# jpl-x/x_multi_agent

Measured on AMD Instinct MI355X. Metric: EKF updates/sec (window=30, 400 MSCKF feats), higher is better.
Workload: dtype f64; 1 GPU; BASELINE.json configs[3]: one agent per GPU, window N=30, K=400 MSCKF tracks (L=N), M=0 SLAM features, n=195; CI payload all-gather every 10 updates; n_poses_max=30, m_slam=0, agents=1, ci_every=10, payload_bytes=306072, ci_tracks_per_round=2, ci_rounds_rank0=0, ci_fused_rank0=0

## Files before the change

### include/xk.h

```cpp
#ifndef XK_H_
#define XK_H_

#ifdef __cplusplus
extern "C" {
#endif

typedef struct xk_handle xk_handle;

typedef enum {
  XK_OK = 0,
  XK_EINVAL = 1,
  XK_ESINGULAR = 2,
  XK_ENAN = 3,
  XK_EDEVICE = 4,
  XK_ENOMEM = 5,
  XK_ECAPACITY = 6
} xk_status;

#define XK_CORE 15


int xk_create(int device, int n_poses_max, int n_feat_max, int k_max, xk_handle **out);
int xk_destroy(xk_handle *h);
const char *xk_strerror(int status);
// ... 101 lines not shown
                       long tag);

int xk_pr_find_candidate(xk_pr *p, int uav_id, const unsigned char *query_vlad, double pr_score_thr, int *index,
                         double *score, long *tag);

int xk_pr_keyframe(xk_pr *p, int index, const double **d_payload, const double **d_tracks, int *n_desc, long *tag,
                   unsigned char *desc_out);

int xk_pr_copy_keyframe(xk_pr *p, int index, double *d_payload_dst, double *d_tracks_dst);

int xk_pr_knn_match(xk_pr *p, const unsigned char *query, int nq, const unsigned char *train, int nt, int *idx, int *dist);

int xk_pr_essential_ransac(xk_pr *p, const float *cur_xy, const float *rec_xy, int n, double fx, double fy, double cx,
                           double cy, double threshold_px, int n_hyp, unsigned long seed, unsigned char *mask,
                           double *E , int *n_inliers);

int xk_pr_essential_hypotheses(xk_pr *p, int first, int count, int *n_cand, double *E ,
                               int *inliers );

typedef struct xk_trk xk_trk;

int xk_trk_create(xk_handle *h, int max_matches, double fx, double fy, double cx, double cy, double s, xk_trk **out);
void xk_trk_destroy(xk_trk *t);

int xk_trk_undistort(xk_trk *t, const double *dist_xy, int n, double *xy);

int xk_trk_fundamental_ransac(xk_trk *t, const float *prev_xy, const float *cur_xy, int n, double threshold_px, int n_hyp,
                              unsigned long seed, unsigned char *mask, double *F ,
                              int *n_inliers);

int xk_trk_fundamental_hypotheses(xk_trk *t, int first, int count, int *n_cand, double *F ,
                                  int *inliers );

int xk_trk_filter_matches(xk_trk *t, const double *prev_dist_xy, const double *cur_dist_xy, int n, double threshold_px,
                          int n_hyp, unsigned long seed, unsigned char *mask, int *keep_idx, double *prev_xy, double *cur_xy,
                          int *n_inliers);


int xk_trk_klt_setup(xk_trk *t, int width, int height, int win_w, int win_h, int max_level, int max_iter, double eps,
                     double min_eig_thr);
int xk_trk_klt_levels(xk_trk *t);

int xk_trk_push_image(xk_trk *t, const unsigned char *img, int stride);

int xk_trk_track(xk_trk *t, const float *prev_xy, int n, double *cur_xy, unsigned char *status, double *min_eig, int *keep_idx,
                 double *kept_prev_xy, double *kept_cur_xy, int *n_kept);

int xk_trk_klt_level(xk_trk *t, int which, int level, unsigned char *img, short *dIx, short *dIy, int *w, int *h);

int xk_build_compress_async(xk_handle *h, double sigma_img);

int xk_build_compress_update_async(xk_handle *h, double sigma_img);

int xk_build_compress_update_pass_async(xk_handle *h, double sigma_img, const double *corr_total, int cov_update);
int xk_fetch_flags(xk_handle *h, int *inlier_msckf, double *gamma_msckf, int *inlier_slam, double *gamma_slam);


int xk_stage_range(xk_handle *h, double range, double img_x_n, double img_y_n, const int facet[3], double sigma_range);
int xk_stage_sun_angle(xk_handle *h, const double q_xyzw[4], double x_angle_deg, double y_angle_deg, const double *calib);
int xk_fetch_aux_flags(xk_handle *h, int *range_inlier, double *range_gamma);
int xk_aux_rows(xk_handle *h, double *H, int ldh, double *res, double *r_diag, int *rows);

int xk_apply_ci_resident(xk_handle *h, const double *ci_P, int ldc, int n, const double *H, int ldh, int m,
                         const double *res, const double *S, int lds, double *correction);

int xk_snapshot_P(xk_handle *h, int restore);


#define XK_NSTAGE 6
typedef struct {
  float total_ms;
  float stage_ms[XK_NSTAGE];
  int stage_launches[XK_NSTAGE];
  char stage_name[XK_NSTAGE][32];
  int n, c1, k_tracks, rows_stacked, n_leaf, n_levels;
} xk_timing;

int xk_bench_staged(xk_handle *h, double sigma_img, int warmup, int steps, xk_timing *out);

int xk_run_steps(xk_handle *h, double sigma_img, int steps);

int xk_caqr_status(const xk_handle *h, int *schedule, int *armed, int *giveups, int *last_reason);

int xk_set_option(xk_handle *h, const char *name, int value);

#ifdef __cplusplus
}
#endif
#endif
```

### x_multi_agent_amd/csrc/xk_api.hip

```cpp
#include "../../include/xk.h"
#ifdef XK_LAB
#include "../../include/xk_lab.h"
#endif

#include <hip/hip_runtime.h>

#include <algorithm>
#include <cmath>
#include <cstdio>
#include <cstdlib>
#include <cstring>
#include <functional>
#include <vector>

#include "xk_chi2_table.h"
#include "xk_feature.hip.h"
#include "xk_slaminit.hip.h"
#include "xk_linalg.hip.h"
#include "xk_caqr_pipe.hip.h"
#include "xk_ci.hip.h"
#include "xk_ciw.hip.h"
#include "xk_ciw_round.hip.h"
#include "xk_aux.hip.h"

// ... 54 lines not shown
  h->CM = round_up(h->n + 1 + 3, 16);
  h->LDA = h->CM + round_up(h->n + 1, 16);
  HIPCHK(h, hipSetDevice(device));
  HIPCHK(h, hipStreamCreateWithFlags(&h->stream, hipStreamNonBlocking));
  HIPCHK(h, hipStreamCreateWithFlags(&h->copy_stream, hipStreamNonBlocking));
  HIPCHK(h, hipEventCreateWithFlags(&h->ev_flags, hipEventDisableTiming));
  HIPCHK(h, hipEventCreateWithFlags(&h->ev_flags_done, hipEventDisableTiming));
  for (auto &e : h->ev) HIPCHK(h, hipEventCreate(&e));
  const size_t nn = (size_t)h->n * h->n;
  h->obs_cap = (size_t)k_max * n_poses_max;
  HIPCHK(h, dalloc(&h->d_q, 7 * (size_t)n_poses_max));
  HIPCHK(h, hipMalloc((void **)&h->d_done_cnt, sizeof(unsigned)));
  HIPCHK(h, hipMemset(h->d_done_cnt, 0, sizeof(unsigned)));
  h->h_win = (double *)calloc(7 * (size_t)n_poses_max, sizeof(double));
  if (!h->h_win) return fail(h, XK_EDEVICE, "host allocation");
  h->d_p = h->d_q + 4 * (size_t)n_poses_max;
  HIPCHK(h, dalloc(&h->d_obs, 2 * h->obs_cap + ((size_t)k_max + 2) / 2 + 1));
  h->d_trk_off = (int *)(h->d_obs + 2 * h->obs_cap);
  HIPCHK(h, dalloc(&h->d_feat, 3 * (size_t)n_feat_max));
  HIPCHK(h, dalloc(&h->d_zlast, 2 * (size_t)n_feat_max));
  HIPCHK(h, dalloc(&h->d_anchor, (size_t)n_feat_max));
  HIPCHK(h, dalloc(&h->d_tsz, (size_t)n_feat_max));
  HIPCHK(h, dalloc(&h->d_P, nn));
  HIPCHK(h, dalloc(&h->d_Pout, nn));
  HIPCHK(h, dalloc(&h->d_fq, (size_t)450));
  HIPCHK(h, dalloc(&h->d_chi95, (size_t)XK_CHI2_LEN));
  HIPCHK(h, dalloc(&h->d_chi90, (size_t)XK_CHI2_LEN));
  HIPCHK(h, hipMemcpy(h->d_chi95, XK_CHI2_095, sizeof(double) * XK_CHI2_LEN, hipMemcpyHostToDevice));
  HIPCHK(h, hipMemcpy(h->d_chi90, XK_CHI2_090, sizeof(double) * XK_CHI2_LEN, hipMemcpyHostToDevice));
  HIPCHK(h, dalloc(&h->d_A, ((size_t)h->ntiles_max * h->DB + 256) * h->C1P));
  HIPCHK(h, hipMemset(h->d_A + (size_t)h->ntiles_max * h->DB * h->C1P, 0, sizeof(double) * 256 * h->C1P));
  h->hc_stride = xk_hc_stride(h->DB, h->C1P);
  h->opt_hlite = env_int("XK_HLITE", 1);
  h->rows_compact = false;
  HIPCHK(h, dalloc(&h->d_Hc, (size_t)std::max(k_max, 1) * h->hc_stride));
  HIPCHK(h, dalloc(&h->d_tile_rows, (size_t)h->ntiles_max));
  for (auto &pp : h->d_panel) HIPCHK(h, dalloc(&pp, (size_t)(h->ntiles_max + 10) * 256));
  HIPCHK(h, dalloc(&h->d_inl, (size_t)k_max));
  HIPCHK(h, dalloc(&h->d_inl_s, (size_t)n_feat_max));
  HIPCHK(h, dalloc(&h->d_gn, (size_t)k_max));
  HIPCHK(h, dalloc(&h->d_gam, (size_t)k_max));
  HIPCHK(h, dalloc(&h->d_gam_s, (size_t)n_feat_max));
  HIPCHK(h, dalloc(&h->d_gpf, 3 * (size_t)k_max));
  HIPCHK(h, dalloc(&h->d_R, (size_t)h->C1P * h->C1P));
  HIPCHK(h, hipMemset(h->d_R, 0, sizeof(double) * (size_t)h->C1P * h->C1P));
  HIPCHK(h, dalloc(&h->d_R2, (size_t)(h->C1P + 32) * h->C1P));
  HIPCHK(h, hipMemset(h->d_R2, 0, sizeof(double) * (size_t)(h->C1P + 32) * h->C1P));
  {
    hipDeviceProp_t prop;
    HIPCHK(h, hipGetDeviceProperties(&prop, device));
    h->n_cu = prop.multiProcessorCount;
    h->persist_ok = h->DB == 64 && h->C1 <= XkPipeWide::COLS && h->n_cu == 256;
    if (h->persist_ok) {
      int nb1 = 0;
      const void *kfn = h->C1 <= XkPipeNarrow::COLS ? (const void *)xk_caqr_pipe<XkPipeNarrow> : (const void *)xk_caqr_pipe<XkPipeWide>;
      if (hipOccupancyMaxActiveBlocksPerMultiprocessor(&nb1, kfn, XK_PIPE_THREADS, 0) != hipSuccess) nb1 = 0;
      h->persist_ok = nb1 >= 1;
      if (h->persist_ok && h->C1 <= XkPipeNarrow::COLS) {
        int nb2 = 0;
        if (hipOccupancyMaxActiveBlocksPerMultiprocessor(&nb2, (const void *)xk_caqr_pipe<XkPipeNarrow2>, XK_PIPE_THREADS, 0) != hipSuccess) nb2 = 0;
        if (nb2 < 1) h->opt_split = -1;
      }
      (void)hipGetLastError();
    }
    h->fast_capable = h->persist_ok;
    h->tail_capable = h->DB == 128 && h->n_cu == 256 && h->C1 > 32;
    if (h->tail_capable) {
      int nbt = 0, nbt4 = 0;
      if (hipOccupancyMaxActiveBlocksPerMultiprocessor(&nbt, (const void *)xk_caqr_pipe<XkPipeTail>, XK_PIPE_THREADS, 0) != hipSuccess) nbt = 0;
      if (hipOccupancyMaxActiveBlocksPerMultiprocessor(&nbt4, (const void *)xk_caqr_pipe<XkPipeTail4>, XK_PIPE_THREADS, 0) != hipSuccess) nbt4 = 0;
      h->tail_capable = nbt >= 1 && nbt4 >= 1;
      (void)hipGetLastError();
    }
    h->tail_ok = h->tail_capable;
    h->opt_tail = env_int("XK_CAQR_TAIL", 1);
    h->opt_slam_split = env_int("XK_SLAM_SPLIT", 1);
    h->opt_pipe_min_rows = env_int("XK_PIPE_MIN_ROWS", 1);
    h->rearm_after = env_int("XK_CAQR_REARM", 64);
    h->opt_resident = env_int("XK_CAQR_RESIDENT", 1);
    h->opt_poison = env_int("XK_CAQR_RESIDENT_POISON", 0);
    h->opt_test_stall = env_int("XK_CAQR_TEST_STALL", 0);
    h->opt_tall26 = env_int("XK_CAQR_TALL26", 1);
    h->opt_kalman = env_int("XK_PIPE_KALMAN", 1);
    if (h->opt_split >= 0) h->opt_split = env_int("XK_PIPE_SPLIT", 1);
    if (!h->fast_capable && h->DB == 64 && h->C1 <= XkPipeWide::COLS) {
      snprintf(h->err, sizeof(h->err), "single-launch CAQR unavailable on device %d: %s; the multi-launch schedule serves every update",
               device, h->n_cu != 256 ? "the process does not see 256 compute units (partition mode or CU mask)"
                                      : "a 768-thread workgroup of the kernel does not fit a compute unit");
      static const int quiet = env_int("XK_QUIET", 0);
      if (!quiet) fprintf(stderr, "xk: %s (n_cu = %d)\n", h->err, h->n_cu);
    }
    if (h->persist_ok || h->tail_capable) {
      const size_t np = h->persist_ok ? (size_t)(h->C1 + 15) / 16 : (size_t)XkPipeTail4::COLS / 16, strips = np * XK_PIPE_RLS;
      h->xslab_doubles = strips * 16 * h->C1P * 2 + strips * 256;
      HIPCHK(h, dalloc(&h->d_x1, 2 * h->xslab_doubles));
      HIPCHK(h, hipMemsetD32Async((hipDeviceptr_t)h->d_x1, (int)(XK_NOTYET_BITS & 0xffffffffu), 2 * 2 * h->xslab_doubles, h->stream));
      HIPCHK(h, dalloc(&h->d_rs, (size_t)8 * XK_PIPE_NT_MAX * 16 * h->C1P));
      HIPCHK(h, dalloc(&h->d_rpb, (size_t)8 * XK_PIPE_NT_MAX * 256));
      HIPCHK(h, dalloc(&h->d_xsync, (size_t)2 * XP_WORDS * 16));
      HIPCHK(h, hipMemset(h->d_xsync, 0, sizeof(unsigned) * 2 * XP_WORDS * 16));
      h->xsync_phase = 0;
#ifdef XK_LAB
      HIPCHK(h, dalloc(&h->d_pdbg, (size_t)XK_PDBG_WORDS));
      HIPCHK(h, hipMemset(h->d_pdbg, 0, sizeof(long long) * XK_PDBG_WORDS));
#endif
    }
  }
  HIPCHK(h, dalloc(&h->d_Maug, (size_t)h->CM * h->LDA));
  HIPCHK(h, dalloc(&h->d_X, (size_t)h->CM * h->LDA));
  HIPCHK(h, dalloc(&h->d_corr, (size_t)h->n + 4));
  HIPCHK(h, dalloc(&h->d_ct, (size_t)h->n));
  HIPCHK(h, dalloc(&h->d_tmpH, (size_t)h->CM * h->n));
  HIPCHK(h, dalloc(&h->d_tmpS, (size_t)h->CM * h->CM));
  HIPCHK(h, dalloc(&h->d_tmpP, nn));
  HIPCHK(h, dalloc(&h->d_rdiag, (size_t)h->CM));
  HIPCHK(h, dalloc(&h->d_tmpz, (size_t)h->CM));
  HIPCHK(h, dalloc(&h->d_aux, 3 * ((size_t)h->n + 1) + 8));
  HIPCHK(h, dalloc(&h->d_Taug, (size_t)h->CM * ((size_t)h->n + 2)));
  HIPCHK(h, hipHostMalloc((void **)&h->h_out, sizeof(double) * ((size_t)h->n + 4), hipHostMallocDefault));
  memset(h->h_out, 0, sizeof(double) * ((size_t)h->n + 4));
  h->d_status = (int *)(h->h_out + h->n);
  HIPCHK(h, dalloc(&h->d_payload, (size_t)xk_payload_doubles(n_poses_max, n_feat_max)));
  HIPCHK(h, dalloc(&h->d_ci, (size_t)4 * nn + 64 * (size_t)h->n + 1024));
  HIPCHK(h, dalloc(&h->d_ciw, (size_t)XK_CIW_WS));
  h->h_pin_doubles = nn + 8 * (size_t)h->n + 4 * (size_t)k_max + 4 * (size_t)n_feat_max + 1024;
  HIPCHK(h, hipHostMalloc((void **)&h->h_pin, sizeof(double) * h->h_pin_doubles));
  h->csr_cap = 24 * (size_t)h->n + 3 * (size_t)n_feat_max * h->n;
  {
    const size_t m = (size_t)std::max(n_feat_max, 1);
    HIPCHK(h, dalloc(&h->d_trk2_off, m + 1));
    HIPCHK(h, dalloc(&h->d_inl2, m));
    HIPCHK(h, dalloc(&h->d_gn2, m));
    HIPCHK(h, dalloc(&h->d_obs2, 2 * m * n_poses_max));
    HIPCHK(h, dalloc(&h->d_gpf2, 3 * m));
    HIPCHK(h, dalloc(&h->d_W2, m * h->DB * h->na));
    HIPCHK(h, dalloc(&h->d_gam2, m));
    HIPCHK(h, dalloc(&h->d_H1, 3 * m * h->n));
    HIPCHK(h, dalloc(&h->d_H2, 9 * m));
    HIPCHK(h, dalloc(&h->d_r1, 3 * m));
    HIPCHK(h, dalloc(&h->d_feat2, 3 * m));
    h->h_trk2_off = (int *)calloc(m + 1, sizeof(int));
    if (!h->h_trk2_off) return fail(h, XK_ENOMEM, "host track offsets");
  }
  HIPCHK(h, dalloc(&h->d_csr_v, h->csr_cap + XK_CORE * XK_CORE + 9 * (size_t)n_feat_max * n_feat_max + 7 * (size_t)n_poses_max + ((size_t)h->n + 2 + h->csr_cap) / 2 + 1));
  h->d_csr_i = nullptr;
  h->h_trk_off = (int *)calloc((size_t)k_max + 1, sizeof(int));
  if (!h->h_trk_off) return fail(h, XK_ENOMEM, "host track offsets");
  HIPCHK(h, hipHostMalloc((void **)&h->h_pin_i, sizeof(int) * ((size_t)k_max + n_feat_max + 512)));
  h->stage_bytes = std::max({sizeof(double) * 2 * h->obs_cap + sizeof(int) * ((size_t)k_max + 1), sizeof(double) * 7 * (size_t)n_poses_max,
                             (sizeof(int) + sizeof(double)) * h->csr_cap + sizeof(int) * ((size_t)h->n + 1) + sizeof(double) * (XK_CORE * XK_CORE + 9 * (size_t)n_feat_max * n_feat_max + 7 * (size_t)n_poses_max),
                             sizeof(double) * 8 * (size_t)std::max(n_feat_max, 1)}) + 256;
  for (auto &sp : h->h_stage) HIPCHK(h, hipHostMalloc((void **)&sp, h->stage_bytes));

  HIPCHK(h, hipHostMalloc((void **)&h->h_flag_i, sizeof(int) * ((size_t)k_max + n_feat_max + 8)));
  HIPCHK(h, hipHostMalloc((void **)&h->h_flag_d, sizeof(double) * ((size_t)k_max + n_feat_max + 8)));
  memset(h->d_status, 0, sizeof(int) * 4);
  HIPCHK(h, hipMemset(h->d_tile_rows, 0, sizeof(int) * (size_t)h->ntiles_max));
  h->sigma_img = 0.0;
  *out = h;
  return XK_OK;
}

extern "C" int xk_destroy(xk_handle *h) {
  if (!h) return XK_OK;
  hipSetDevice(h->device);
  hipStreamSynchronize(h->stream);
// ... 1942 lines not shown
    hipError_t e = hipStreamEndCapture(h->stream, &g);
    if (rc != XK_OK) return rc;
    if (e != hipSuccess) return fail(h, XK_EDEVICE, "graph capture", e);
    HIPCHK(h, hipGraphInstantiate(&ge, g, nullptr, nullptr, 0));
    for (int it = 0; it < steps; ++it) HIPCHK(h, hipGraphLaunch(ge, h->stream));
    rc = read_status(h);
    hipGraphExecDestroy(ge);
    hipGraphDestroy(g);
    return rc;
  }
#endif
  for (int attempt = 0; attempt < 2; ++attempt) {
    for (int it = 0; it < steps; ++it) {
      int rc = launch_build(h, sigma_img, attempt > 0 || it > 0);
      if (rc != XK_OK) return rc;
      UpdateSpec u = compressed_spec(h, nullptr, 1);
      rc = launch_compress(h, nullptr, &u);
      if (rc != XK_OK) return rc;
      if (!h->last.fused) rc = launch_update(h, u);
      if (rc != XK_OK) return rc;
    }
    const int rc = read_status(h, attempt == 0);
    if (rc != XK_RETRY_CLASSIC) return rc;
  }
  return XK_EDEVICE;
}

#ifdef XK_LAB
__global__ __launch_bounds__(256) void xk_probe_mfma(double *out, int iters) {
  xk_d4 a0 = {0, 0, 0, 0}, a1 = a0, a2 = a0, a3 = a0;
  const double x = 1.0 + threadIdx.x * 1e-9, y = 1.0 - threadIdx.x * 1e-9;
  for (int i = 0; i < iters; ++i) {
    a0 = __builtin_amdgcn_mfma_f64_16x16x4f64(x, y, a0, 0, 0, 0);
    a1 = __builtin_amdgcn_mfma_f64_16x16x4f64(y, x, a1, 0, 0, 0);
    a2 = __builtin_amdgcn_mfma_f64_16x16x4f64(x, x, a2, 0, 0, 0);
    a3 = __builtin_amdgcn_mfma_f64_16x16x4f64(y, y, a3, 0, 0, 0);
  }
  out[(size_t)blockIdx.x * blockDim.x + threadIdx.x] = a0[0] + a1[1] + a2[2] + a3[3];
}
__global__ __launch_bounds__(256) void xk_probe_fma(double *out, int iters) {
  double a[8];
  const double x = 1.0 + threadIdx.x * 1e-9, y = 1e-9 * threadIdx.x;
#pragma unroll
  for (int k = 0; k < 8; ++k) a[k] = k;
  for (int i = 0; i < iters; ++i) {
#pragma unroll
    for (int k = 0; k < 8; ++k) a[k] = fma(a[k], x, y);
  }
  double s = 0;
#pragma unroll
  for (int k = 0; k < 8; ++k) s += a[k];
  out[(size_t)blockIdx.x * blockDim.x + threadIdx.x] = s;
}

extern "C" int xk_probe_fp64_peak(xk_handle *h, int use_mfma, double *tflops) {
  if (!h || !tflops) return XK_EINVAL;
  HIPCHK(h, hipSetDevice(h->device));
  const int blocks = 256 * 8, iters = 20000;
  double *buf = nullptr;
  HIPCHK(h, hipMalloc((void **)&buf, sizeof(double) * blocks * 256));
  for (int rep = 0; rep < 2; ++rep) {
    HIPCHK(h, hipEventRecord(h->ev[8], h->stream));
    if (use_mfma) hipLaunchKernelGGL(xk_probe_mfma, dim3(blocks), dim3(256), 0, h->stream, buf, iters);
    else hipLaunchKernelGGL(xk_probe_fma, dim3(blocks), dim3(256), 0, h->stream, buf, iters);
    HIPCHK(h, hipEventRecord(h->ev[9], h->stream));
    HIPCHK(h, hipStreamSynchronize(h->stream));
  }
  float ms = 0;
  hipEventElapsedTime(&ms, h->ev[8], h->ev[9]);
  hipFree(buf);
  const double waves = (double)blocks * 4;
  const double flops = use_mfma ? waves * iters * 4.0 * (2.0 * 16 * 16 * 4) : waves * 64.0 * iters * 8.0 * 2.0;
  *tflops = flops / (ms * 1e-3) / 1e12;
  return XK_OK;
}
#endif

extern "C" int xk_set_option(xk_handle *h, const char *name, int value) {
  if (!h || !name) return XK_EINVAL;
  if (!strcmp(name, "caqr_resident")) h->opt_resident = value;
  else if (!strcmp(name, "caqr_rearm")) h->rearm_after = value;
  else if (!strcmp(name, "caqr_tail")) h->opt_tail = value;
  else if (!strcmp(name, "slam_split")) h->opt_slam_split = value;
  else if (!strcmp(name, "ci_weight_search")) {
    if (value != 0 && value != 1) return fail(h, XK_EINVAL, "xk_set_option: ci_weight_search is 0 or 1");
    h->opt_ci_search = value;
  }
#ifdef XK_LAB
  else if (!strcmp(name, "caqr_poison")) h->opt_poison = value;
  else if (!strcmp(name, "caqr_test_stall")) h->opt_test_stall = value;
  else if (!strcmp(name, "caqr_tall26")) h->opt_tall26 = value;
  else if (!strcmp(name, "pipe_kalman")) h->opt_kalman = value;
  else if (!strcmp(name, "pipe_split")) { if (h->opt_split >= 0) h->opt_split = value; }
  else if (!strcmp(name, "caqr_hlite")) h->opt_hlite = value;
#endif
  else return fail(h, XK_EINVAL, "xk_set_option: unknown option");
  return XK_OK;
}

extern "C" int xk_caqr_status(const xk_handle *h, int *schedule, int *armed, int *giveups, int *last_reason) {
  if (!h) return XK_EINVAL;
  if (schedule) *schedule = outcome_status(h->last);
  if (armed) *armed = (h->persist_ok || h->tail_ok) ? 1 : 0;
  if (giveups) *giveups = h->fast_giveups;
  if (last_reason) *last_reason = h->fast_reason;
  return XK_OK;
}

#ifdef XK_LAB
extern "C" int xk_is_lab(void) { return 1; }
extern "C" int xk_debug_persist_stamps(xk_handle *h, long long *out, int n_out) {
  if (!h || !out || !h->d_pdbg) return XK_EINVAL;
  HIPCHK(h, hipSetDevice(h->device));
  HIPCHK(h, hipStreamSynchronize(h->stream));
  HIPCHK(h, hipMemcpy(out, h->d_pdbg, sizeof(long long) * (size_t)std::min(n_out, XK_PDBG_WORDS), hipMemcpyDeviceToHost));
  return XK_OK;
}
extern "C" int xk_debug_feature_points(xk_handle *h, double *gpf, int *gn_iters, int K) {
  if (!h || !gpf || !gn_iters || K < 0 || K != h->K) return XK_EINVAL;
  HIPCHK(h, hipSetDevice(h->device));
  HIPCHK(h, hipStreamSynchronize(h->stream));
  if (K == 0) return XK_OK;
  HIPCHK(h, hipMemcpy(gpf, h->d_gpf, sizeof(double) * 3 * (size_t)K, hipMemcpyDeviceToHost));
  HIPCHK(h, hipMemcpy(gn_iters, h->d_gn, sizeof(int) * (size_t)K, hipMemcpyDeviceToHost));
  return XK_OK;
}
#endif

#if defined(XK_FEAT_PROBE) && defined(XK_LAB)
extern "C" int xk_debug_feature_phases(xk_handle *h, double sigma_img, long long *out, int n_out) {
  const size_t bytes = sizeof(long long) * (size_t)(12 * h->K);
  hipMalloc((void **)&h->feat_dbg, bytes);
  hipMemset(h->feat_dbg, 0, bytes);
  int rc = launch_build(h, sigma_img);
  hipStreamSynchronize(h->stream);
  hipMemcpy(out, h->feat_dbg, std::min(bytes, sizeof(long long) * (size_t)n_out), hipMemcpyDeviceToHost);
  hipFree(h->feat_dbg);
  h->feat_dbg = nullptr;
  return rc;
}
#endif

#include "xk_place.hip.h"
#include "xk_essential.hip.h"

#define XK_PR_MAX_KEYFRAMES 15

struct xk_pr {
  xk_handle *h;
  int k, L, n_nodes, kmax, W, n_words, clusters, VW, max_desc;
  long pay_n, trk_n;
  unsigned int *d_node_desc;
  int *d_children, *d_word_of_node, *d_node_of_word;
  unsigned int *d_vlad;
  unsigned int *d_kfdesc;
  double *d_payload;
  double *d_tracks;
  int n_desc[XK_PR_MAX_KEYFRAMES];
  long tag[XK_PR_MAX_KEYFRAMES];
  std::vector<int> *uav_ids[XK_PR_MAX_KEYFRAMES];
  int order[XK_PR_MAX_KEYFRAMES], live;
  unsigned int *d_q, *d_t, *d_qvlad;
  int *d_ham, *d_knn;
  int *h_int;
  unsigned int *h_words;
  size_t h_words_cap;
  double *d_ess;
  unsigned char *h_ess;
  int ess_n_hyp;
};

#define XK_ESS_OFF_SUM ((size_t)XK_ESS_MAX_HYP * XK_ESS_MAXC * 9)
#define XK_ESS_OFF_E (XK_ESS_OFF_SUM + (size_t)XK_ESS_MAX_HYP * XK_ESS_MAXC)
#define XK_ESS_OFF_KEY (XK_ESS_OFF_E + 9)
#define XK_ESS_DOUBLES (XK_ESS_OFF_KEY + 1)
#define XK_ESS_INTS ((size_t)XK_ESS_MAX_HYP * (XK_ESS_MAXC + 2) + 2)

extern "C" void xk_pr_destroy(xk_pr *p) {
  if (!p) return;
  hipFree(p->d_node_desc); hipFree(p->d_children); hipFree(p->d_word_of_node); hipFree(p->d_node_of_word);
  hipFree(p->d_vlad); hipFree(p->d_kfdesc); hipFree(p->d_payload); hipFree(p->d_tracks);
  hipFree(p->d_q); hipFree(p->d_t); hipFree(p->d_qvlad); hipFree(p->d_ham); hipFree(p->d_knn);
  if (p->h_int) hipHostFree(p->h_int);
  if (p->h_words) hipHostFree(p->h_words);
  hipFree(p->d_ess);
  if (p->h_ess) hipHostFree(p->h_ess);
  for (auto &u : p->uav_ids) delete u;
  free(p);
}

// ... 675 lines not shown
```

### x_multi_agent_amd/csrc/xk_caqr_pipe.hip.h

```cpp
#pragma once
#include <hip/hip_runtime.h>

#include <type_traits>

#include "xk_linalg.hip.h"
#include "xk_xcd_sync.hip.h"

#define XK_PIPE_THREADS 768
#ifndef XK_PIPE_NPH
#define XK_PIPE_NPH 4
#endif
template <int LPC_, int RPL_, int NT_, int NM_, int NCL_, int NCM_ = 1, int RPLS_ = RPL_, int RPLT_ = RPLS_, int NG_ = 1, int NPH_ = XK_PIPE_NPH>
struct XkPipeGeom {
  static constexpr int LPC = LPC_, RPL = RPL_, NT = NT_, NM = NM_, NCL = NCL_, NCM = NCM_, NG = NG_;
  static constexpr int NPH = NPH_;
  static_assert(NPH_ == 1 || NPH_ == 2 || NPH_ == 4, "XP_TQ_CNT / XP_X1_CNT hold four phases");
  static constexpr int NTG = (NT_ + NG_ - 1) / NG_, NMG = NM_ / NG_;
  static_assert(NM_ % NG_ == 0 && NG_ >= 1 && NG_ <= 2, "first-level groups share the first-level workgroups evenly");
  static constexpr int RPLS = RPLS_, RPLT = RPLT_;
  static_assert(RPLS_ % 4 == 0 && RPLS_ >= 16 && RPLS_ <= RPL_ && RPLT_ % 4 == 0 && RPLT_ >= 16 && RPLT_ <= RPLS_, "the lighter tile steps");
  static constexpr int RM = (NTG + 2) & ~1;
  static constexpr int RL = 8 * NG_;
  static constexpr int COLS = XK_PIPE_THREADS / LPC_;
  static constexpr int ROWS = 8 * NT_ * LPC_ * RPL_;
// ... 15 lines not shown
#ifndef XK_PIPE_TAIL
#define XK_PIPE_TAIL 8, 44, 23, 8, 1, 1, 44, 44, 1, 4
#endif
using XkPipeTail = XkPipeGeom<XK_PIPE_TAIL>;
#ifndef XK_PIPE_TAIL4
#define XK_PIPE_TAIL4 4, 44, 23, 8, 1, 1, 44, 44, 1, 4
#endif
using XkPipeTail4 = XkPipeGeom<XK_PIPE_TAIL4>;
#define XK_PIPE_RLS 16
#define XK_PIPE_NT_MAX 23
#define XK_PIPE_ROWS_MAX 24320
#define XK_PIPE_SLOTS_MAX 1536
#ifndef XK_PIPE_PB
#define XK_PIPE_PB 0, 4, 8, 12, 16
#endif
#ifndef XK_PIPE_PB2
#define XK_PIPE_PB2 0, 8, 16
#endif
template <int NPH>
__host__ __device__ constexpr int xk_pbn(int q) {
  if (NPH == 4) {
    constexpr int t[] = {XK_PIPE_PB};
    return q <= 0 ? 0 : (q >= 4 ? 16 : t[q]);
  }
  if (NPH == 2) {
    constexpr int t[] = {XK_PIPE_PB2};
    return q <= 0 ? 0 : (q >= 2 ? 16 : t[q]);
  }
  return q * (16 / NPH);
}
#ifndef XK_PIPE_ARRD
#define XK_PIPE_ARRD 1
#endif
#ifndef XK_PIPE_PF
#define XK_PIPE_PF 0
#endif
#ifndef XK_PIPE_LOCALLD
#define XK_PIPE_LOCALLD 0
#endif
#if XK_PIPE_LOCALLD
#define XK_LD_LOC(p) xk_ld_grp(p)
#ifdef XK_PIPE_NOINV
#define XK_INV_LOC()
#else
#define XK_INV_LOC() xk_inv_l1()
#endif
#else
#define XK_LD_LOC(p) xk_ld_sc1(p)
#define XK_INV_LOC()
#endif
#ifndef XK_PIPE_TRI
#define XK_PIPE_TRI 0
#endif
#ifndef XK_PIPE_NLW
#define XK_PIPE_NLW 7
#endif
#ifndef XK_PIPE_CHUNK
#define XK_PIPE_CHUNK 0
#endif

enum {
  XP_CENSUS = 0,
  XP_ABORT = 9,
  XP_TQ_CNT = 16,
  XP_MB_CNT = 48,
  XP_X1_CNT = 64,
  XP_P_CNT = 64 + 4 * XK_CAQR_MAXP,
  XP_R_CNT = 64 + 5 * XK_CAQR_MAXP,
  XP_WORDS = 64 + 6 * XK_CAQR_MAXP
};

struct XkCaqrPipeArgs {
  const double *A;
  const double *Hc;
  int hs, nhc;
  const int *tile_rows;
  int nslots;
  int slot_rows;
  int lead_stride;
  int res_col;
  int nextra;
  long extra_row0;
  int C1P, C1;
  double *Rout;
  double *S;
  double *PB;
  double *X1, *X1P;
  double *X2;
  double *Xnext;
  long xnext_doubles;
  unsigned *sync, *sync_next;
  int *status;
  long long *dbg;
  int test_stall;
  int acc_tag;
  int kal, kn;
  const double *Pin;
  double *Pout;
  double sigma2;
  double *corr;
  const double *ct;
  unsigned long long *done_flag;
  unsigned long long done_seq;
};
typedef const XkCaqrPipeArgs __attribute__((address_space(4))) *XkPipeArgsPtr;
__device__ __forceinline__ XkCaqrPipeArgs xk_pipe_args(XkPipeArgsPtr ap) {
  XkCaqrPipeArgs a;
  __builtin_memcpy(&a, (const void *)ap, sizeof(a));
  return a;
}

__device__ __forceinline__ void xk_pipe_arrive(unsigned *cnt) {
  (void)__hip_atomic_fetch_add(cnt, 1u, XK_ARRIVE_ORDER, __HIP_MEMORY_SCOPE_AGENT);
}
__device__ __forceinline__ int xk_launder(int v) {
  asm volatile("" : "+v"(v));
  return v;
}
__device__ __forceinline__ size_t xk_blk(int c, int r) { return (size_t)(c >> 2) * 64 + (size_t)r * 4 + (size_t)(c & 3); }
__device__ __forceinline__ int xk_pipe_srccol(const XkCaqrPipeArgs &a, int c) { return (a.res_col > 0 && c == a.C1 - 1) ? a.res_col : c; }
__device__ __forceinline__ void xk_pipe_lastcut(int trail, int NCL, int &ncl, int &lchalf, int &lsplit) {
  ncl = (NCL > 1 && trail > 32 * XK_PIPE_NLW) ? NCL : 1;
  lchalf = max(4, 4 * ((trail + 4 * XK_PIPE_NLW * ncl - 1) / (4 * XK_PIPE_NLW * ncl)));
  lsplit = max(1, (trail + lchalf - 1) / lchalf);
}
__device__ __forceinline__ bool xk_pipe_wait(unsigned *word, unsigned target, unsigned *ab, unsigned reason, unsigned *s_ok) {
  if (threadIdx.x == 0) *s_ok = xk_spin_ge(word, target, ab, reason) ? 1u : 0u;
  __syncthreads();
  const bool ok = *s_ok != 0u;
  XK_ACQUIRE_FENCE();
  __syncthreads();
  return ok;
}

__device__ __forceinline__ int xk_pipe_wait_phases(unsigned *cnt0, int stride, int q, int nph, unsigned target, unsigned *ab, unsigned reason,
                                                   unsigned *s_ok) {
  if (threadIdx.x == 0) {
    unsigned av = 0;
    if (xk_spin_ge(cnt0 + (size_t)q * stride, target, ab, reason)) {
      av = (unsigned)q + 1u;
      while ((int)av < nph && __hip_atomic_load(cnt0 + (size_t)av * stride, XK_RLX_AGENT) >= target) ++av;
    }
    *s_ok = av;
  }
  __syncthreads();
  const int av = (int)*s_ok;
  XK_ACQUIRE_FENCE();
  __syncthreads();
  return av;
}

template <int KK, int LPC, int RPL>
__device__ __forceinline__ void xk_pipe_tapply(double (&b)[RPL], int rel, bool live, int part, const double *ubuf, const double *sc) {
  if constexpr (XK_PIPE_CHUNK || RPL > 32) {
    constexpr int RPLP = RPL + 2, H = RPL / 4;
    constexpr int pb = KK & 1;
    const xk_d2 *useg = reinterpret_cast<const xk_d2 *>(ubuf + (pb * LPC + part) * RPLP);
    const double mtt = sc[pb * 4];
    if (rel > KK && live && mtt != 0.0) {
      double d0 = 0.0, d1 = 0.0, d2 = 0.0, d3 = 0.0;
      {
        xk_d2 u[H];
#pragma unroll
        for (int r = 0; r < H; ++r) u[r] = useg[r];
#pragma unroll
        for (int r = 0; r < H; ++r) {
          if (r & 1) { d2 = fma(u[r][0], b[2 * r], d2); d3 = fma(u[r][1], b[2 * r + 1], d3); }
          else { d0 = fma(u[r][0], b[2 * r], d0); d1 = fma(u[r][1], b[2 * r + 1], d1); }
        }
      }
      xk_d2 v[H];
#pragma unroll
      for (int r = 0; r < H; ++r) v[r] = useg[H + r];
#pragma unroll
      for (int r = 0; r < H; ++r) {
        if ((H + r) & 1) { d2 = fma(v[r][0], b[2 * (H + r)], d2); d3 = fma(v[r][1], b[2 * (H + r) + 1], d3); }
        else { d0 = fma(v[r][0], b[2 * (H + r)], d0); d1 = fma(v[r][1], b[2 * (H + r) + 1], d1); }
      }
      const double w = mtt * xk_group_sum<LPC>((d0 + d1) + (d2 + d3));
#pragma unroll
      for (int r = 0; r < H; ++r) {
        b[2 * (H + r)] = fma(w, v[r][0], b[2 * (H + r)]);
        b[2 * (H + r) + 1] = fma(w, v[r][1], b[2 * (H + r) + 1]);
      }
      const xk_d2 *useg2 = useg + xk_launder(0);
#pragma unroll
      for (int r = 0; r < H; ++r) {
        const xk_d2 u = useg2[r];
        b[2 * r] = fma(w, u[0], b[2 * r]);
        b[2 * r + 1] = fma(w, u[1], b[2 * r + 1]);
      }
    }
  } else {
// ... 144 lines not shown
struct XkNoStepHook { __device__ __forceinline__ void operator()(int) const {} };
template <int LPC, int K, int K1, int KH, int RPL, typename Hook, typename Every>
__device__ __forceinline__ void xk_pipe_range_it(double (&b)[RPL], double (*b2)[RPL], int rel, bool live, bool live2, int part, int nsteps,
                                                 double *ubuf, double *sc, bool hook_on, Hook hook, Every every) {
  if constexpr (K < K1) {
    if (K < nsteps) {
      xk_pipe_apply2<LPC, K - 1, RPL>(b, b2, rel, live, live2, part, ubuf, sc);
      xk_pipe_form<LPC, K, RPL>(b, rel, part, ubuf, sc);
      if (K == KH && hook_on) asm volatile("s_waitcnt vmcnt(0)" ::: "memory");
      __syncthreads();
      if (K == KH && hook_on && threadIdx.x == 0) hook();
      every(K);
    } else if (K == nsteps) {
      xk_pipe_apply2<LPC, K - 1, RPL>(b, b2, rel, live, live2, part, ubuf, sc);
    }
    xk_pipe_range_it<LPC, K + 1, K1, KH, RPL>(b, b2, rel, live, live2, part, nsteps, ubuf, sc, hook_on, hook, every);
  }
}
template <int LPC, int K0, int K1, int KH, int RPL, typename Hook, typename Every>
__device__ __forceinline__ void xk_pipe_range(double (&b)[RPL], double (*b2)[RPL], int rel, bool live, bool live2, int part, int nsteps,
                                              double *ubuf, double *sc, bool hook_on, Hook hook, Every every) {
  if (K0 < nsteps) xk_pipe_form<LPC, K0, RPL>(b, rel, part, ubuf, sc);
  if (KH == K0 && hook_on) asm volatile("s_waitcnt vmcnt(0)" ::: "memory");
  __syncthreads();
  if (KH == K0 && hook_on && threadIdx.x == 0) hook();
  every(K0);
  xk_pipe_range_it<LPC, K0 + 1, K1, KH, RPL>(b, b2, rel, live, live2, part, nsteps, ubuf, sc, hook_on, hook, every);
  if (nsteps >= K1) xk_pipe_apply2<LPC, K1 - 1, RPL>(b, b2, rel, live, live2, part, ubuf, sc);
}
template <int LPC, int K0, int K1, int KH, int RPL, typename Hook>
__device__ __forceinline__ void xk_pipe_range(double (&b)[RPL], double (*b2)[RPL], int rel, bool live, bool live2, int part, int nsteps,
                                              double *ubuf, double *sc, bool hook_on, Hook hook) {
  xk_pipe_range<LPC, K0, K1, KH, RPL>(b, b2, rel, live, live2, part, nsteps, ubuf, sc, hook_on, hook, XkNoStepHook());
}

template <class G>
__device__ __forceinline__ int xk_pipe_rowplan(const XkCaqrPipeArgs &a, int j, int *pre, int *myrows, int *rows_accepted) {
  constexpr int NTP = 8 * G::NT, CAP = G::LPC * G::RPL;
  const int tid = threadIdx.x, lane = tid & 63, wave = tid >> 6;
  __shared__ int wsum[XK_PIPE_THREADS / 64];
  int carry = 0;
  for (int base = 0; base < a.nslots; base += XK_PIPE_THREADS) {
    const int t = base + tid;
    int v = t < a.nslots ? a.tile_rows[t] : 0;
    if (a.lead_stride > 0 && t < a.nslots && t % a.lead_stride == 0) v = max(v, 32);
#pragma unroll
    for (int o = 1; o < 64; o <<= 1) {
      const int u = __shfl_up(v, o, 64);
      if (lane >= o) v += u;
    }
    if (lane == 63) wsum[wave] = v;
    __syncthreads();
    int off = carry;
    for (int w = 0; w < wave; ++w) off += wsum[w];
    if (t < a.nslots) pre[t + 1] = v + off;
    int tot = 0;
    for (int w = 0; w < XK_PIPE_THREADS / 64; ++w) tot += wsum[w];
    carry += tot;
    __syncthreads();
  }
  if (tid == 0) pre[0] = 0;
  const int Rs = carry, R = Rs + a.nextra, TR = (R + NTP - 1) / NTP;
  *rows_accepted = R;
  __syncthreads();
  if (TR > CAP) return 0;
  if (tid < CAP) {
    const int g = j * TR + tid;
    int phys = -1;
    if (tid < TR && g >= Rs && g < R) phys = (int)a.extra_row0 + (g - Rs);
    else if (tid < TR && g < Rs) {
      int lo = 0, hi = a.nslots;
      while (hi - lo > 1) {
        const int mid = (lo + hi) >> 1;
        if (pre[mid] <= g) lo = mid; else hi = mid;
      }
      phys = lo * a.slot_rows + (g - pre[lo]);
    }
    myrows[tid] = phys;
  }
  __syncthreads();
  return max(TR, 1);
}

template <class G, int RPL>
__device__ __noinline__ bool xk_pipe_tile(XkPipeArgsPtr ap, int xcc, int slot, long long t_entry, double *ubuf, double *sc, unsigned *s_ok,
                                          const int *myrows, double *hbuf, int hcap_doubles, int nvalid) {
  constexpr int NT = G::NT, LPC = G::LPC, NPH = G::NPH, GS = 16 / NPH, ARRD = XK_PIPE_ARRD;
  static_assert(ARRD < xk_pbn<NPH>(1) && ARRD < 16 - xk_pbn<NPH>(NPH - 1), "a phase is counted in before the next one is published");
  const XkCaqrPipeArgs a = xk_pipe_args(ap);
  unsigned *sync = a.sync, *ab = sync + XP_ABORT * 16;
  const int tid = threadIdx.x;
  const int j = xcc * NT + slot;
  const int cabs = tid / LPC, part_ = tid % LPC;
  const bool mine = cabs < a.C1;
  const int npanels = (a.C1 + 15) / 16;
  const bool stamp = a.dbg && xcc == 0 && slot == 1 && tid == 0;
  double b[RPL];
  if (a.nhc > 0) {
    constexpr int BR = 8, CG = XK_PIPE_THREADS / LPC;
    const int hs = a.hs, C1P = a.C1P, ccl = min(cabs, C1P - 1);
    double *Tb = hbuf, *recs = hbuf + LPC * BR * C1P;
    const int hcap = (hcap_doubles - LPC * BR * C1P) / hs;
#pragma unroll
    for (int r = 0; r < RPL; ++r) b[r] = 0.0;
    if (stamp) a.dbg[1544] = wall_clock64();
    const int s_lo = myrows[0] >> 6, s_hi = nvalid > 0 ? myrows[nvalid - 1] >> 6 : -1;
    const int fp = __builtin_amdgcn_readfirstlane(tid / CG), fc = tid % CG;
    if (stamp) a.dbg[1545] = wall_clock64();
    for (int lo = max(s_lo, 0); lo <= s_hi && lo < a.nhc; lo += hcap) {
      const int hi = min(min(lo + hcap, s_hi + 1), a.nhc);
      {
        const xk_d2 *src = reinterpret_cast<const xk_d2 *>(a.Hc + (size_t)lo * hs);
        xk_d2 *dst = reinterpret_cast<xk_d2 *>(recs);
        const int tot = (hi - lo) * (hs / 2);
        for (int base = 0; base < tot; base += 6 * XK_PIPE_THREADS) {
          xk_d2 t[6];
#pragma unroll
          for (int i = 0; i < 6; ++i) t[i] = src[min(base + i * XK_PIPE_THREADS + tid, tot - 1)];
#pragma unroll
          for (int i = 0; i < 6; ++i) {
            const int e = base + i * XK_PIPE_THREADS + tid;
            if (e < tot) dst[e] = t[i];
          }
        }
      }
      __syncthreads();
      if (stamp) a.dbg[1546] = wall_clock64();
      int kcur = -1, r0 = -2;
      double nw0 = 0.0, nw1 = 0.0, nw2 = 0.0, wres = 0.0, x0 = 0.0, x1 = 0.0;
      const bool whole = lo <= s_lo && s_hi < hi;
#pragma unroll
      for (int rb = 0; rb < (RPL + BR - 1) / BR; ++rb) {
        if (fc < C1P) {
#pragma unroll
          for (int j = 0; j < BR; ++j) {
            if (rb * BR + j < RPL) {
              const int ph = __builtin_amdgcn_readfirstlane(myrows[fp * RPL + rb * BR + j]), sl = ph >> 6;
              if (ph >= 0 && sl >= lo && sl < hi) {
                const double *rec = recs + (sl - lo) * hs;
                if (sl != kcur) {
                  const xk_d2 *wc = reinterpret_cast<const xk_d2 *>(rec + XK_HC_VR + XK_HC_WC * xk_pipe_srccol(a, fc));
                  const xk_d2 q0 = wc[0], q1 = wc[1], q2 = wc[2];
                  nw0 = -q0[0]; nw1 = -q0[1]; nw2 = -q1[0]; x0 = q1[1]; x1 = q2[0]; r0 = (int)q2[1];
                  wres = (r0 == -1) ? 1.0 : 0.0;
                  kcur = sl;
                }
                const int rr = (ph & 63) + 3, dd = rr - r0;
                const xk_d2 va = reinterpret_cast<const xk_d2 *>(rec + 4 * rr)[0], vb = reinterpret_cast<const xk_d2 *>(rec + 4 * rr)[1];
                const double add = (dd == 0) ? x0 : ((dd == 1) ? x1 : 0.0);
                Tb[(fp * BR + j) * C1P + fc] = fma(wres, vb[1], fma(nw2, vb[0], fma(nw1, va[1], nw0 * va[0]))) + add;
              }
            }
          }
        }
        __syncthreads();
        if (whole) {
#pragma unroll
          for (int j = 0; j < BR; ++j) {
            if (rb * BR + j < RPL) {
              const double v = Tb[(part_ * BR + j) * C1P + ccl];
              b[rb * BR + j] = (mine && part_ * RPL + rb * BR + j < nvalid) ? v : 0.0;
            }
          }
        } else {
#pragma unroll
          for (int j = 0; j < BR; ++j) {
            if (rb * BR + j < RPL) {
              const int ph = myrows[part_ * RPL + rb * BR + j], sl = ph >> 6;
              const double v = Tb[(part_ * BR + j) * C1P + ccl];
              if (ph >= 0 && sl >= lo && sl < hi) b[rb * BR + j] = mine ? v : 0.0;
            }
          }
        }
        __syncthreads();
        if (stamp) a.dbg[1547 + rb] = wall_clock64();
      }
    }
    if (s_hi >= a.nhc) {
      const double *Ac = a.A + xk_pipe_srccol(a, ccl);
#pragma unroll
      for (int h0 = 0; h0 < RPL; h0 += 16) {
        double x[16];
#pragma unroll
        for (int r = 0; r < 16; ++r) {
          if (h0 + r < RPL) x[r] = Ac[(size_t)max(myrows[part_ * RPL + h0 + r], 0) * C1P];
        }
#pragma unroll
        for (int r = 0; r < 16; ++r) {
          if (h0 + r < RPL) {
            const int ph = myrows[part_ * RPL + h0 + r];
            if (mine && ph >= 0 && (ph >> 6) >= a.nhc) b[h0 + r] = x[r];
          }
        }
      }
    }
  } else
  {
    int pr[RPL];
#pragma unroll
    for (int r = 0; r < RPL; ++r) pr[r] = myrows[part_ * RPL + r];
    const double *Ac = a.A + xk_pipe_srccol(a, min(cabs, a.C1P - 1));
#pragma unroll
    for (int h0 = 0; h0 < RPL; h0 += 16) {
      double x[16];
#pragma unroll
      for (int r = 0; r < 16; ++r) {
        if (h0 + r < RPL) x[r] = Ac[(size_t)max(pr[h0 + r], 0) * a.C1P];
      }
#pragma unroll
      for (int r = 0; r < 16; ++r) {
        if (h0 + r < RPL) b[h0 + r] = (mine && pr[h0 + r] >= 0) ? x[r] : 0.0;
      }
    }
  }
  double *myS = a.S + (size_t)j * 16 * a.C1P;
  double *myPB = a.PB + (size_t)j * 256;
  if (stamp) { a.dbg[1536] = t_entry; a.dbg[1537] = wall_clock64(); }
  for (int k = 0; k < npanels; ++k) {
    const int c0 = 16 * k;
    const int part = xk_launder(part_);
    const int rel = xk_launder(cabs) - c0;
    const int nsteps = (a.C1 - c0 < 16) ? a.C1 - c0 : 16;
    const bool full = nsteps == 16;
    const int wrel = (tid >> 6) * (64 / LPC) - c0;
    const bool hot = wrel <= 0 && wrel > -(64 / LPC);
    const bool pub = mine && part == 0 && rel >= 0;
    const unsigned epoch = (unsigned)(k + 1);
    if (stamp) { a.dbg[16 * k + 0] = wall_clock64(); a.dbg[16 * k + 8] = clock64(); }
    if (a.dbg && slot == 0 && tid == 0) a.dbg[12288 + xcc * 32 + k] = wall_clock64();
    if (a.dbg && tid == 0 && k < 2) a.dbg[40960 + 256 * k + j] = wall_clock64();
    if (a.dbg && tid == 0 && k == 0) a.dbg[40960 + 512 + j] = t_entry;
    if (hot) __builtin_amdgcn_s_setprio(3);
    auto phase = [&](auto qc) {
      constexpr int q = decltype(qc)::value;
      auto hook = [&]() { xk_pipe_arrive(sync + (XP_TQ_CNT + (q - 1) * 8 + xcc) * 16); if (a.dbg && k == 0 && q == 1) a.dbg[47104 + j] = wall_clock64(); };
      xk_pipe_range<LPC, xk_pbn<NPH>(q), xk_pbn<NPH>(q + 1), (q > 0 ? xk_pbn<NPH>(q) + ARRD : -1), RPL>(b, nullptr, rel, mine, false, part, nsteps, ubuf, sc, full, hook);
      if (pub) {
        if (rel < 16) {
          double *pb = xk_opaque(myPB + xk_blk(rel, 0));
#pragma unroll
          for (int r = xk_pbn<NPH>(q); r < xk_pbn<NPH>(q + 1); ++r) pb[r * 4] = (r > rel) ? 0.0 : b[r];
        } else {
          double *ps = xk_opaque(myS + xk_blk(cabs, 0));
#pragma unroll
          for (int r = xk_pbn<NPH>(q); r < xk_pbn<NPH>(q + 1); ++r) ps[r * 4] = b[r];
        }
      }
      if (stamp && q < 4) a.dbg[16 * k + 1 + q] = wall_clock64();
    };
    phase(std::integral_constant<int, 0>{});
    if constexpr (NPH >= 2) phase(std::integral_constant<int, 1>{});
    if constexpr (NPH >= 4) { phase(std::integral_constant<int, 2>{}); phase(std::integral_constant<int, 3>{}); }
    if constexpr (NPH >= 8) {
      phase(std::integral_constant<int, 4>{}); phase(std::integral_constant<int, 5>{});
      phase(std::integral_constant<int, 6>{}); phase(std::integral_constant<int, 7>{});
    }
    if (hot) __builtin_amdgcn_s_setprio(0);
    if (stamp) { a.dbg[16 * k + 9] = clock64(); a.dbg[16 * k + 10] = wall_clock64(); }
    asm volatile("s_waitcnt vmcnt(0)" ::: "memory");
    __syncthreads();
    if (tid == 0) {
      for (int q = full ? NPH - 1 : 0; q < NPH; ++q)
        xk_pipe_arrive(sync + (XP_TQ_CNT + q * 8 + xcc) * 16);
    }
    if (stamp) a.dbg[16 * k + 5] = wall_clock64();
    if (k + 1 == npanels) break;
    if (!xk_pipe_wait(sync + (XP_MB_CNT + xcc) * 16, (unsigned)G::NM * epoch, ab, 2u, s_ok)) return false;
    if (stamp) a.dbg[16 * k + 6] = wall_clock64();
    XK_INV_LOC();
    if (mine && rel >= 16 && part == 0) {
      const double *ps = xk_opaque(myS + xk_blk(cabs, 0));
#pragma unroll
      for (int r = 0; r < 16; ++r) b[r] = XK_LD_LOC(ps + r * 4);
    }
    if (stamp) {
      double sink = 0;
      for (int r = 0; r < 16; ++r) sink += b[r];
      asm volatile("" ::"v"(sink));
      a.dbg[16 * k + 7] = wall_clock64();
    }
  }
  if (stamp) a.dbg[1538] = wall_clock64();
  return true;
}

__device__ __forceinline__ void xk_lds_dma16(const double *src, unsigned lds_byte) {
  asm volatile("s_mov_b32 m0, %1\n\tglobal_load_lds_dwordx4 %0, off sc1" ::"v"(src), "s"(lds_byte) : "memory", "m0");
}

template <class G>
__device__ __noinline__ bool xk_pipe_first(XkPipeArgsPtr ap, int xcc, int item, double *ubuf, double *sc, unsigned *s_ok, double *pfbuf) {
  constexpr int NT = G::NT, NM = G::NMG, RM = G::RM, NP = 16, NPH = G::NPH, GS = 16 / NPH, NCL = G::NCL, NCM = G::NCM;
  constexpr int NG = G::NG, NTG = G::NTG;
  const XkCaqrPipeArgs a = xk_pipe_args(ap);
  unsigned *sync = a.sync, *ab = sync + XP_ABORT * 16;
  const int tid = threadIdx.x;
  const int cidx_ = tid / NP, part_ = tid & (NP - 1);
  const bool panel = cidx_ < 16;
  const int npanels = (a.C1 + 15) / 16;
  const int grp = NG > 1 ? item / NM : 0;
  item -= grp * NM;
  const int nts = NG > 1 ? min(NTG, NT - grp * NTG) : NT;
  const int base = xcc * NT + grp * NTG;
  const bool has_pending = !(xcc == 0 && grp == 0);
  const size_t SS = (size_t)16 * a.C1P;
  const bool stamp = a.dbg && xcc == 0 && item == 0 && tid == 0;
  for (int k = 0; k < npanels; ++k) {
    const int c0 = 16 * k, trail = max(0, a.C1 - c0 - 16);
    const int cidx = xk_launder(cidx_), part = xk_launder(part_);
    const int mh = min(32, 4 * ((trail + 4 * NM * NCM - 1) / (4 * NM * NCM))), mch = mh * NCM;
    const bool active = item == 0 || item * mch < trail;
    const int col = panel ? c0 + cidx : c0 + 16 + item * mch + (cidx - 16);
    const int col2 = col + mh;
    const bool mine = active && col < a.C1 && (panel || cidx - 16 < mh);
    const bool mine2 = NCM > 1 && active && !panel && cidx - 16 < mh && col2 < a.C1;
    const int nsteps = (a.C1 - c0 < 16) ? a.C1 - c0 : 16;
    const bool full = nsteps == 16;
    const unsigned epoch = (unsigned)(k + 1);
    const size_t slab = (size_t)k * XK_PIPE_RLS + xcc * NG + grp;
    double b[RM], b2[NCM > 1 ? RM : 2];
    b[0] = 0.0;
    b2[0] = 0.0;
    int ncl_prev, lchalf_prev, lsplit_prev;
    xk_pipe_lastcut(a.C1 - c0, NCL, ncl_prev, lchalf_prev, lsplit_prev);
    lsplit_prev = min(XK_PIPE_NLW, lsplit_prev);
    const size_t pslab = (size_t)(k - 1) * XK_PIPE_RLS + xcc * NG + grp;
    if (k >= 1 && has_pending) {
#if XK_DATA_POLL
      double pb1[1] = {0.0}, pb2[1] = {0.0};
      if (!xk_poll_slots<1>(pb1, a.X2 + pslab * SS + xk_blk(min(col, a.C1P - 1), part), 0, mine, ab, 4u)) *s_ok = 0u;
      if constexpr (NCM > 1) {
        if (!xk_poll_slots<1>(pb2, a.X2 + pslab * SS + xk_blk(min(col2, a.C1P - 1), part), 0, mine2, ab, 4u)) *s_ok = 0u;
      }
      __syncthreads();
      if (*s_ok == 0u) return false;
      if (mine) b[0] = pb1[0];
      if constexpr (NCM > 1) b2[0] = mine2 ? pb2[0] : 0.0;
      if (a.dbg && tid == 0) a.dbg[4096 + ((xcc * NG + grp) * NM + item) * 32 + k] = wall_clock64();
#else
      if (!xk_pipe_wait(sync + (XP_P_CNT + k - 1) * 16, (unsigned)lsplit_prev, ab, 4u, s_ok)) return false;
      if (mine) b[0] = xk_ld_sc1(a.X2 + pslab * SS + xk_blk(col, part));
#endif
    }
#pragma unroll
    for (int s = 1; s < RM; ++s) b[s] = 0.0;
    if constexpr (NCM > 1) {
#pragma unroll
      for (int s = 1; s < RM; ++s) b2[s] = 0.0;
#if !XK_DATA_POLL
      if (k >= 1 && has_pending && mine2) b2[0] = xk_ld_sc1(a.X2 + pslab * SS + xk_blk(col2, part));
#endif
    }
    double *g02 = a.S + (size_t)base * SS + xk_blk(min(col2, a.C1P - 1), part);
    double *x12 = a.X1 + slab * SS + xk_blk(min(col2, a.C1P - 1), part);
    const size_t lane_off = panel ? xk_blk(cidx, part) : xk_blk(col, part);
    const size_t strip_step = panel ? 256 : SS;
    double *g0 = (panel ? a.PB + (size_t)base * 256 : a.S + (size_t)base * SS) + lane_off;
    double *x1 = panel ? a.X1P + slab * 256 + xk_blk(cidx, part) : a.X1 + slab * SS + xk_blk(col, part);
    const bool x1_mine = mine && (!panel || item == 0);
    bool ok = true;
    int loaded = 0;
    constexpr bool PF = XK_PIPE_PF && NG == 1 && NCM == 1 && NPH == 4 && NT <= 24 && xk_pbn<NPH>(1) == 4 && xk_pbn<NPH>(2) == 8 && xk_pbn<NPH>(3) == 12;
    const int ln = tid & 63, cid4 = cidx & ~3;
    const int wcol = panel ? c0 + cid4 : c0 + 16 + item * mch + (cid4 - 16);
    const bool wv_ok = active && (panel || cid4 - 16 < mh) && wcol < a.C1;
    double *pfw = pfbuf + (size_t)(tid >> 6) * (24 * 16);
    const unsigned pfw_lds = (unsigned)__builtin_amdgcn_readfirstlane((int)(unsigned)(size_t)pfw);
    const double *pfsrc = (panel ? a.PB + (size_t)base * 256 + xk_blk(cid4, 0) : a.S + (size_t)base * SS + xk_blk(wcol, 0)) +
                          (size_t)(ln >> 3) * strip_step + (ln & 7) * 2;
    auto phase = [&](auto qc) {
      constexpr int q = decltype(qc)::value;
      if (!ok) return;
#ifdef XK_PIPE_PROBE_M1PACE
      if (q > 0 && loaded > q) {
        if (xk_pipe_wait_phases(sync + (XP_TQ_CNT + xcc) * 16, 8 * 16, q, NPH, (unsigned)NT * epoch, ab, 6u, s_ok) == 0) { ok = false; return; }
      }
#endif
      if (loaded <= q) {
#ifdef XK_PIPE_PROBE_M1ALL
        int av = xk_pipe_wait_phases(sync + (XP_TQ_CNT + xcc) * 16, 8 * 16, q, NPH, (unsigned)NT * epoch, ab, 6u, s_ok);
        if (av != 0) av = NPH;
#else
        const int av = xk_pipe_wait_phases(sync + (XP_TQ_CNT + xcc) * 16, 8 * 16, q, NPH, (unsigned)NT * epoch, ab, 6u, s_ok);
#endif
        if (av == 0) { ok = false; return; }
        if (stamp && q < 4) a.dbg[512 + 16 * k + 2 * q] = wall_clock64();
        if (a.dbg && tid == 0 && k == 0 && q == 0) a.dbg[46080 + (xcc * NG + grp) * NM + item] = wall_clock64();
        XK_INV_LOC();
        if constexpr (PF) {
          for (int p = loaded; p < av; ++p) {
            if (wv_ok) {
              const double *src = pfsrc + (size_t)p * 16;
#pragma unroll
              for (int j = 0; j < 3; ++j)
                if (8 * j + (ln >> 3) < NT) xk_lds_dma16(src + (size_t)(8 * j) * strip_step, pfw_lds + (unsigned)j * 1024u);
              asm volatile("s_waitcnt vmcnt(0)" ::: "memory");
              if (mine && part >= p * GS && part < (p + 1) * GS) {
                typedef const __attribute__((address_space(3))) double xk_lds_cd;
                xk_lds_cd *pl = (xk_lds_cd *)(pfw + (part - p * GS) * 4 + (cidx & 3));
#pragma unroll
                for (int s = 1; s <= NT; ++s) b[s] = pl[(s - 1) * 16];
              }
              if (p + 1 < av) asm volatile("s_waitcnt lgkmcnt(0)" ::: "memory");
            }
          }
        } else {
          if (active && mine && part >= xk_pbn<NPH>(loaded) && part < xk_pbn<NPH>(av)) {
            double *g = xk_opaque(g0);
#pragma unroll
            for (int s = 1; s <= NTG; ++s)
              if (NG == 1 || s <= nts) b[s] = XK_LD_LOC(g + (size_t)(s - 1) * strip_step);
          }
        }
        if constexpr (NCM > 1) {
          if (mine2 && part >= xk_pbn<NPH>(loaded) && part < xk_pbn<NPH>(av)) {
            double *g = xk_opaque(g02);
#pragma unroll
            for (int s = 1; s <= NTG; ++s)
              if (NG == 1 || s <= nts) b2[s] = xk_ld_sc1(g + (size_t)(s - 1) * SS);
          }
        }
        loaded = av;
#ifdef XK_PIPE_M1PROBE
        asm volatile("s_waitcnt vmcnt(0)" ::: "memory");
        if (stamp && q < 4) a.dbg[512 + 16 * k + 10 + q] = wall_clock64();
#endif
      }
      if (!active) return;
      if (panel) __builtin_amdgcn_s_setprio(3);
      auto hook = [&]() { xk_pipe_arrive(sync + (XP_X1_CNT + (q - 1) * XK_CAQR_MAXP + k) * 16); };
      if constexpr (NCM > 1)
        xk_pipe_range<0, xk_pbn<NPH>(q), xk_pbn<NPH>(q + 1), (q > 0 ? xk_pbn<NPH>(q) : -1), RM>(b, &b2, cidx, mine, mine2, part, nsteps, ubuf, sc, full && !XK_DATA_POLL, hook);
      else
        xk_pipe_range<0, xk_pbn<NPH>(q), xk_pbn<NPH>(q + 1), (q > 0 ? xk_pbn<NPH>(q) : -1), RM>(b, nullptr, cidx, mine, false, part, nsteps, ubuf, sc, full && !XK_DATA_POLL, hook);
      if (panel) __builtin_amdgcn_s_setprio(0);
      if (q < NPH - 1 && x1_mine && part >= xk_pbn<NPH>(q) && part < xk_pbn<NPH>(q + 1)) xk_st_sc1(x1, (panel && part > cidx) ? 0.0 : b[0]);
      if constexpr (NCM > 1) {
        if (q < NPH - 1 && mine2 && part >= xk_pbn<NPH>(q) && part < xk_pbn<NPH>(q + 1)) xk_st_sc1(x12, b2[0]);
      }
      if (stamp && q < 4) a.dbg[512 + 16 * k + 2 * q + 1] = wall_clock64();
      if (a.dbg && tid == 0 && q == 0) a.dbg[4096 + ((xcc * NG + grp) * NM + item) * 32 + 16 + k] = wall_clock64();
      if (a.dbg && tid == 0 && q < 4) a.dbg[16640 + (((xcc * NG + grp) * NM + item) * 16 + k) * 4 + q] = wall_clock64();
    };
    phase(std::integral_constant<int, 0>{});
    if constexpr (NPH >= 2) phase(std::integral_constant<int, 1>{});
    if constexpr (NPH >= 4) { phase(std::integral_constant<int, 2>{}); phase(std::integral_constant<int, 3>{}); }
    if constexpr (NPH >= 8) {
      phase(std::integral_constant<int, 4>{}); phase(std::integral_constant<int, 5>{});
      phase(std::integral_constant<int, 6>{}); phase(std::integral_constant<int, 7>{});
    }
    if (!ok) return false;
    if (mine) {
      if (!panel) {
        double *g = xk_opaque(g0);
#pragma unroll
        for (int s = 1; s <= NTG; ++s)
          if (NG == 1 || s <= nts) g[(size_t)(s - 1) * strip_step] = b[s];
      }
      if (x1_mine && part >= xk_pbn<NPH>(NPH - 1)) xk_st_sc1(x1, (panel && part > cidx) ? 0.0 : b[0]);
    }
    if constexpr (NCM > 1) {
      if (mine2) {
        double *g = xk_opaque(g02);
#pragma unroll
        for (int s = 1; s <= NTG; ++s)
          if (NG == 1 || s <= nts) g[(size_t)(s - 1) * SS] = b2[s];
        if (part >= xk_pbn<NPH>(NPH - 1)) xk_st_sc1(x12, b2[0]);
      }
    }
    asm volatile("s_waitcnt vmcnt(0)" ::: "memory");
    __syncthreads();
    if (tid == 0) {
      xk_pipe_arrive(sync + (XP_MB_CNT + xcc) * 16);
      if (!XK_DATA_POLL)
        for (int q = (full && active) ? NPH - 1 : 0; q < NPH; ++q) xk_pipe_arrive(sync + (XP_X1_CNT + q * XK_CAQR_MAXP + k) * 16);
    }
    if (stamp) a.dbg[512 + 16 * k + 8] = wall_clock64();
  }
  return true;
}

template <class G>
__device__ __noinline__ bool xk_pipe_last(XkPipeArgsPtr ap, int lidx, double *ubuf, double *sc, unsigned *s_ok) {
  constexpr int NP = 16, RL = G::RL, NPH = G::NPH, GS = 16 / NPH, NCL = G::NCL, NM = G::NM;
  const XkCaqrPipeArgs a = xk_pipe_args(ap);
  unsigned *sync = a.sync, *ab = sync + XP_ABORT * 16;
  const int tid = threadIdx.x;
  const int cidx_ = tid / NP, part_ = tid & (NP - 1);
  const bool panel = cidx_ < 16;
  const int npanels = (a.C1 + 15) / 16;
  const bool stamp = a.dbg && lidx == 0 && tid == 0;
  const size_t SS = (size_t)16 * a.C1P;
  for (int k = 0; k < npanels; ++k) {
    const int c0 = 16 * k, trail = max(0, a.C1 - c0 - 16);
    int ncl, lchalf, lsplit;
    xk_pipe_lastcut(trail, NCL, ncl, lchalf, lsplit);
    if (lidx >= lsplit || lidx >= XK_PIPE_NLW) continue;
    const int cidx = xk_launder(cidx_), part = xk_launder(part_);
    const int col = panel ? c0 + cidx : c0 + 16 + lidx * lchalf + (cidx - 16);
    const int col2 = col + XK_PIPE_NLW * lchalf;
    const bool mine = col < a.C1 && (panel || cidx - 16 < lchalf);
    const bool mine2 = ncl > 1 && !panel && cidx - 16 < lchalf && col2 < a.C1;
    const int nsteps = (a.C1 - c0 < 16) ? a.C1 - c0 : 16;
    const double *src = panel ? a.X1P + (size_t)k * XK_PIPE_RLS * 256 + xk_blk(cidx, part) : a.X1 + (size_t)k * XK_PIPE_RLS * SS + xk_blk(col, part);
    const double *src2 = a.X1 + (size_t)k * XK_PIPE_RLS * SS + xk_blk(min(col2, a.C1P - 1), part);
    const size_t sstep = panel ? 256 : SS;
    double b[RL], b2[RL];
#pragma unroll
    for (int s = 0; s < RL; ++s) { b[s] = 0.0; b2[s] = 0.0; }
    bool ok = true;
    int loaded = 0;
    auto phase = [&](auto qc) {
      constexpr int q = decltype(qc)::value;
      if (!ok || nsteps <= xk_pbn<NPH>(q)) return;
#if XK_DATA_POLL
      {
        const bool rows_q = part >= xk_pbn<NPH>(q) && part < xk_pbn<NPH>(q + 1);
        bool got = xk_poll_slots<RL>(b, src, sstep, rows_q && mine, ab, 5u);
        if (got && ncl > 1) got = xk_poll_slots<RL>(b2, src2, SS, rows_q && mine2, ab, 5u);
        if (!got) *s_ok = 0u;
        __syncthreads();
        if (*s_ok == 0u) { ok = false; return; }
        if (stamp && q < 4) a.dbg[1024 + 16 * k + 2 * q] = wall_clock64();
        if (a.dbg && tid == 0 && q < 2) a.dbg[8192 + lidx * 64 + 16 * q + k] = wall_clock64();
        if (a.dbg && tid == 0 && q < 4) a.dbg[32768 + ((lidx * 16 + k) * 4 + q) * 2] = wall_clock64();
        (void)loaded;
      }
#else
      if (loaded <= q) {
        const int av = xk_pipe_wait_phases(sync + (XP_X1_CNT + k) * 16, XK_CAQR_MAXP * 16, q, NPH, 8u * NM, ab, 5u, s_ok);
        if (av == 0) { ok = false; return; }
        if (stamp && q < 4) a.dbg[1024 + 16 * k + 2 * q] = wall_clock64();
        if (part >= xk_pbn<NPH>(loaded) && part < xk_pbn<NPH>(av)) {
          if (mine) {
#pragma unroll
            for (int s = 0; s < RL; ++s) b[s] = xk_ld_sc1(src + s * sstep);
          }
          if (mine2) {
#pragma unroll
            for (int s = 0; s < RL; ++s) b2[s] = xk_ld_sc1(src2 + s * SS);
          }
        }
        loaded = av;
      }
#endif
      if (panel) __builtin_amdgcn_s_setprio(3);
      xk_pipe_range<0, xk_pbn<NPH>(q), xk_pbn<NPH>(q + 1), -1, RL>(b, ncl > 1 ? &b2 : nullptr, panel ? cidx : 16, mine, mine2, part, nsteps, ubuf, sc, false, []() {});
      if (panel) __builtin_amdgcn_s_setprio(0);
      if (stamp && q < 4) a.dbg[1024 + 16 * k + 2 * q + 1] = wall_clock64();
      if (a.dbg && tid == 0 && q < 4) a.dbg[32768 + ((lidx * 16 + k) * 4 + q) * 2 + 1] = wall_clock64();
    };
    phase(std::integral_constant<int, 0>{});
    if constexpr (NPH >= 2) phase(std::integral_constant<int, 1>{});
    if constexpr (NPH >= 4) { phase(std::integral_constant<int, 2>{}); phase(std::integral_constant<int, 3>{}); }
    if (!ok) return false;
    auto rout = [&](size_t at, double v) { if (a.kal) xk_st_sc1(a.Rout + at, v); else a.Rout[at] = v; };
    if (mine) {
      if (panel) {
        if (lidx == 0 && c0 + part < a.C1) rout((size_t)(c0 + part) * a.C1P + xk_pipe_srccol(a, col), (part > cidx) ? 0.0 : b[0]);
      } else {
        if (k + 1 < npanels) {
          double *dst = a.X2 + (size_t)k * XK_PIPE_RLS * SS + xk_blk(col, part);
#pragma unroll
          for (int s = 1; s < RL; ++s) xk_st_sc1(dst + s * SS, b[s]);
        }
        if (c0 + part < a.C1) rout((size_t)(c0 + part) * a.C1P + xk_pipe_srccol(a, col), b[0]);
      }
    }
    if (mine2) {
      if (k + 1 < npanels) {
        double *dst = a.X2 + (size_t)k * XK_PIPE_RLS * SS + xk_blk(col2, part);
#pragma unroll
        for (int s = 1; s < RL; ++s) xk_st_sc1(dst + s * SS, b2[s]);
      }
      if (c0 + part < a.C1) rout((size_t)(c0 + part) * a.C1P + xk_pipe_srccol(a, col2), b2[0]);
    }
    asm volatile("s_waitcnt vmcnt(0)" ::: "memory");
    __syncthreads();
    if (tid == 0) {
      if (!XK_DATA_POLL && k + 1 < npanels) xk_pipe_arrive(sync + (XP_P_CNT + k) * 16);
      if (a.kal) xk_pipe_arrive(sync + (XP_R_CNT + k) * 16);
    }
    if (stamp) a.dbg[1024 + 16 * k + 8] = wall_clock64();
    if (a.dbg && tid == 0) a.dbg[8192 + lidx * 64 + 32 + k] = wall_clock64();
  }
  if (stamp) a.dbg[1539] = wall_clock64();
  return true;
}


#define XK_KAL_NB 12
#define XK_KAL_DC 207
#define XK_KAL_TLD 226
#define XK_KAL_LDS (16 * XK_KAL_TLD + 13 * 288 + 13 * 256 + 13 * 256 + 12 * 256 + 256 + 256 + 16 * 17 + 16)
typedef __attribute__((address_space(3))) double xk_ldsd;
struct XkKalLds {
  xk_ldsd *Tl, *Wt, *part, *Pc, *P0, *W12s, *dbuf, *Ls, *zcol, *Sp, *Xs;
  __device__ __forceinline__ explicit XkKalLds(xk_ldsd *base) {
    Tl = base; Wt = Tl + 16 * XK_KAL_TLD; part = Wt + 13 * 288; Pc = part + 13 * 256; P0 = Pc + 13 * 256; W12s = P0 + 12 * 256;
    dbuf = W12s + 256; Ls = dbuf + 256; zcol = Ls + 16 * 17;
    Sp = Wt;
    Xs = part;
  }
};
template <int NPIV>
__device__ __forceinline__ bool xk_kal_chol16(const xk_ldsd *blk, xk_ldsd *linv, int lane) {
  const int tt = lane & 15;
  double v[16], w[16];
#pragma unroll
  for (int q = 0; q < 16; ++q) { v[q] = blk[16 * tt + q]; w[q] = (tt == q) ? 1.0 : 0.0; }
  bool bad = false;
  xk_chol16_step<0>(v, w, bad); xk_chol16_step<1>(v, w, bad); xk_chol16_step<2>(v, w, bad); xk_chol16_step<3>(v, w, bad);
  if constexpr (NPIV > 4) {
    xk_chol16_step<4>(v, w, bad); xk_chol16_step<5>(v, w, bad); xk_chol16_step<6>(v, w, bad); xk_chol16_step<7>(v, w, bad);
    xk_chol16_step<8>(v, w, bad); xk_chol16_step<9>(v, w, bad); xk_chol16_step<10>(v, w, bad); xk_chol16_step<11>(v, w, bad);
    xk_chol16_step<12>(v, w, bad); xk_chol16_step<13>(v, w, bad); xk_chol16_step<14>(v, w, bad); xk_chol16_step<15>(v, w, bad);
  }
  if (lane < 16) {
#pragma unroll
    for (int q = 0; q < 16; ++q) linv[q * 17 + tt] = w[q];
  }
  return bad;
}
template <bool REG, int NQ>
__device__ __forceinline__ void xk_kal_downdate(const XkKalLds &m, xk_d4 (&Pt)[XK_KAL_NB], const xk_d4 &X, int wave, int lane) {
  constexpr int NB = XK_KAL_NB;
  const xk_ldsd *xl = m.Xs + lane;
  xk_ldsd *p0 = m.P0 + lane;
#pragma unroll
  for (int I = 0; I < NB; ++I) {
    double xc[NQ];
    xk_d4 c;
#pragma unroll
    for (int q = 0; q < NQ; ++q) xc[q] = xl[I * 256 + 64 * q];
#pragma unroll
    for (int r = 0; r < 4; ++r) c[r] = REG ? Pt[I][r] : p0[I * 256 + 64 * r];
#pragma unroll
    for (int q = 0; q < NQ; ++q) c = __builtin_amdgcn_mfma_f64_16x16x4f64(-xc[q], X[q], c, 0, 0, 0);
    if (REG) Pt[I] = c;
    else {
#pragma unroll
      for (int r = 0; r < 4; ++r) p0[I * 256 + 64 * r] = c[r];
    }
    __builtin_amdgcn_sched_barrier(0);
  }
  xk_d4 c12, ccc;
#pragma unroll
  for (int r = 0; r < 4; ++r) { c12[r] = m.Pc[wave * 256 + 64 * r + lane]; ccc[r] = REG ? 0.0 : m.Pc[12 * 256 + 64 * r + lane]; }
#pragma unroll
  for (int q = 0; q < NQ; ++q) {
    c12 = __builtin_amdgcn_mfma_f64_16x16x4f64(-X[q], xl[12 * 256 + 64 * q], c12, 0, 0, 0);
    if (!REG) ccc = __builtin_amdgcn_mfma_f64_16x16x4f64(-xl[12 * 256 + 64 * q], xl[12 * 256 + 64 * q], ccc, 0, 0, 0);
  }
#pragma unroll
  for (int r = 0; r < 4; ++r) { m.Pc[wave * 256 + 64 * r + lane] = c12[r]; if (!REG) m.Pc[12 * 256 + 64 * r + lane] = ccc[r]; }
}
template <bool REG>
__device__ __forceinline__ void xk_kal_block(const XkKalLds &m, xk_d4 (&Pt)[XK_KAL_NB], int k, int nrows, int n, double sigma2, int wave, int lane,
                                             bool &bad, long long *stp) {
#define XK_KSTAMP(i) do { if (stp && lane == 0) stp[i] = wall_clock64(); } while (0)
  constexpr int NB = XK_KAL_NB, TLD = XK_KAL_TLD;
  const int li = lane & 15, lk = lane >> 4;
  const int nq = (nrows + 3) >> 2;
  const xk_ldsd *ta = m.Tl + li * TLD + lk;
  const xk_ldsd *p0 = m.P0 + lane;
  xk_d4 w0 = {0, 0, 0, 0}, w1 = {0, 0, 0, 0};
#define XK_KAL_WTILE(I)                                                                                                   \
  {                                                                                                                       \
    double ac[4], bc[4];                                                                                                  \
    _Pragma("unroll") for (int q = 0; q < 4; ++q) { ac[q] = ta[16 * (I) + 4 * q]; bc[q] = REG ? Pt[I][q] : p0[(I) * 256 + 64 * q]; } \
    _Pragma("unroll") for (int q = 0; q < 4; ++q) {                                                                       \
      if ((I) & 1) w1 = __builtin_amdgcn_mfma_f64_16x16x4f64(ac[q], bc[q], w1, 0, 0, 0);                                  \
      else w0 = __builtin_amdgcn_mfma_f64_16x16x4f64(ac[q], bc[q], w0, 0, 0, 0);                                          \
    }                                                                                                                     \
  }
  switch (k) {
    case 0: XK_KAL_WTILE(0) [[fallthrough]];
    case 1: XK_KAL_WTILE(1) [[fallthrough]];
    case 2: XK_KAL_WTILE(2) [[fallthrough]];
    case 3: XK_KAL_WTILE(3) [[fallthrough]];
    case 4: XK_KAL_WTILE(4) [[fallthrough]];
    case 5: XK_KAL_WTILE(5) [[fallthrough]];
    case 6: XK_KAL_WTILE(6) [[fallthrough]];
    case 7: XK_KAL_WTILE(7) [[fallthrough]];
    case 8: XK_KAL_WTILE(8) [[fallthrough]];
    case 9: XK_KAL_WTILE(9) [[fallthrough]];
    case 10: XK_KAL_WTILE(10) [[fallthrough]];
    default: XK_KAL_WTILE(11)
  }
#undef XK_KAL_WTILE
  if (n > 192) {
#pragma unroll
    for (int q = 0; q < 4; ++q) w1 = __builtin_amdgcn_mfma_f64_16x16x4f64(ta[192 + 4 * q], m.Pc[wave * 256 + 16 * li + 4 * q + lk], w1, 0, 0, 0);
  }
  __builtin_amdgcn_sched_barrier(0);
  XK_KSTAMP(2);
  xk_d4 W = w0 + w1;
  {
    xk_d4 x = {0, 0, 0, 0};
    if (wave >= k) {
#pragma unroll
      for (int q = 0; q < 4; ++q) x = __builtin_amdgcn_mfma_f64_16x16x4f64(ta[16 * wave + 4 * q], m.Pc[wave * 256 + 64 * q + lane], x, 0, 0, 0);
    }
#pragma unroll
    for (int r = 0; r < 4; ++r) m.part[wave * 256 + 64 * r + lane] = x[r];
    if (!REG) {
      xk_d4 y = {0, 0, 0, 0};
#pragma unroll
      for (int q = 0; q < 4; ++q) y = __builtin_amdgcn_mfma_f64_16x16x4f64(ta[192 + 4 * q], m.Pc[12 * 256 + 64 * q + lane], y, 0, 0, 0);
#pragma unroll
      for (int r = 0; r < 4; ++r) m.part[12 * 256 + 64 * r + lane] = y[r];
    }
  }
  auto spart = [&](const xk_d4 &Wc, int J) {
    xk_ldsd *wt = m.Wt + J * 288;
#pragma unroll
    for (int r = 0; r < 4; ++r) wt[(lk + 4 * r) * 18 + li] = Wc[r];
    xk_d4 sacc = {0, 0, 0, 0};
#pragma unroll
    for (int q = 0; q < 4; ++q) sacc = __builtin_amdgcn_mfma_f64_16x16x4f64(wt[li * 18 + 4 * q + lk], ta[16 * J + 4 * q], sacc, 0, 0, 0);
#pragma unroll
    for (int r = 0; r < 4; ++r) m.Sp[J * 288 + 64 * r + lane] = sacc[r];
  };
  __builtin_amdgcn_sched_barrier(0);
  spart(W, wave);
  __builtin_amdgcn_sched_barrier(0);
  XK_KSTAMP(3);
  __syncthreads();
  XK_KSTAMP(4);
  if (REG && wave == 11) {
    xk_d4 W12 = {0, 0, 0, 0};
    for (int w = k; w < 13; ++w)
#pragma unroll
      for (int r = 0; r < 4; ++r) W12[r] += m.part[w * 256 + 64 * r + lane];
    if (li == XK_KAL_DC - 192) {
#pragma unroll
      for (int r = 0; r < 4; ++r) W12[r] -= m.zcol[lk + 4 * r];
    }
#pragma unroll
    for (int r = 0; r < 4; ++r) m.W12s[64 * r + lane] = W12[r];
    spart(W12, 12);
  }
  __syncthreads();
  XK_KSTAMP(5);
  if (!REG) {
    xk_d4 S = {0, 0, 0, 0};
    for (int J = k; J < 13; ++J)
#pragma unroll
      for (int r = 0; r < 4; ++r) S[r] += m.Sp[J * 288 + 64 * r + lane];
#pragma unroll
    for (int r = 0; r < 4; ++r) m.dbuf[16 * (lk + 4 * r) + li] = S[r] + ((lk + 4 * r == li) ? sigma2 : 0.0);
    if (nrows <= 4 ? xk_kal_chol16<4>(m.dbuf, m.Ls, lane) : xk_kal_chol16<16>(m.dbuf, m.Ls, lane)) bad = true;
  }
  XK_KSTAMP(6);
  __syncthreads();
  XK_KSTAMP(7);
  double lv[4];
#pragma unroll
  for (int q = 0; q < 4; ++q) lv[q] = m.Ls[li * 17 + 4 * q + lk];
  xk_d4 X = {0, 0, 0, 0};
#pragma unroll
  for (int q = 0; q < 4; ++q) X = __builtin_amdgcn_mfma_f64_16x16x4f64(lv[q], W[q], X, 0, 0, 0);
#pragma unroll
  for (int r = 0; r < 4; ++r) m.Xs[wave * 256 + 64 * r + lane] = X[r];
  if (REG && wave == 11) {
    xk_d4 X12 = {0, 0, 0, 0};
#pragma unroll
    for (int q = 0; q < 4; ++q) X12 = __builtin_amdgcn_mfma_f64_16x16x4f64(lv[q], m.W12s[64 * q + lane], X12, 0, 0, 0);
#pragma unroll
    for (int r = 0; r < 4; ++r) m.Xs[12 * 256 + 64 * r + lane] = X12[r];
  }
  __syncthreads();
  XK_KSTAMP(8);
  if (nq == 1) xk_kal_downdate<REG, 1>(m, Pt, X, wave, lane);
  else xk_kal_downdate<REG, 4>(m, Pt, X, wave, lane);
  XK_KSTAMP(9);
  __syncthreads();
  XK_KSTAMP(10);
#undef XK_KSTAMP
}

template <class G>
__device__ __noinline__ bool xk_pipe_kalman(XkPipeArgsPtr ap, xk_ldsd *kb, unsigned *s_ok) {
  constexpr int NB = XK_KAL_NB, TLD = XK_KAL_TLD, NCL = G::NCL;
  const XkCaqrPipeArgs a = xk_pipe_args(ap);
  unsigned *sync = a.sync, *ab = sync + XP_ABORT * 16;
  const int tid = threadIdx.x, lane_ = tid & 63, wave = __builtin_amdgcn_readfirstlane(tid >> 6);
  const int n = a.kn, na = a.C1 - 1, npanels = (a.C1 + 15) / 16;
  auto ldsym = [&](int row, int col) {
    if (col == XK_KAL_DC) return (a.ct && row < n) ? -a.ct[row] : 0.0;
    return (row < n && col < n) ? 0.5 * (a.Pin[(size_t)row + (size_t)col * n] + a.Pin[(size_t)col + (size_t)row * n]) : 0.0;
  };
  auto fetch = [&](const XkKalLds &m, int k, int &nrows) -> bool {
    const int c0 = 16 * k;
    nrows = min(16, na - c0);
    int ncl, lchalf, lsplit;
    xk_pipe_lastcut(max(0, a.C1 - c0 - 16), NCL, ncl, lchalf, lsplit);
    if (!xk_pipe_wait(sync + (XP_R_CNT + k) * 16, (unsigned)min(XK_PIPE_NLW, lsplit), ab, 8u, s_ok)) return false;
    double tv[5];
#pragma unroll
    for (int u = 0; u < 5; ++u) {
      const int idx = tid + u * XK_PIPE_THREADS, mr = idx / 208, st = idx - 208 * mr, c = st - 15;
      tv[u] = (idx < 16 * 208 && mr < nrows && c >= c0 && c < na) ? xk_ld_sc1(a.Rout + (size_t)(c0 + mr) * a.C1P + c) : 0.0;
    }
#pragma unroll
    for (int u = 0; u < 5; ++u) {
      const int idx = tid + u * XK_PIPE_THREADS, mr = idx / 208, st = idx - 208 * mr;
      if (idx < 16 * 208) m.Tl[mr * TLD + st] = tv[u];
    }
    if (tid < 16) m.zcol[tid] = (tid < nrows) ? xk_ld_sc1(a.Rout + (size_t)(c0 + tid) * a.C1P + na) : 0.0;
    __syncthreads();
    return true;
  };
  auto publish = [&](const XkKalLds &m, int lane) {
    const int li = lane & 15, lk = lane >> 4;
    if (li == XK_KAL_DC - 192) {
#pragma unroll
      for (int r = 0; r < 4; ++r) {
        m.dbuf[16 * wave + lk + 4 * r] = m.Pc[wave * 256 + 64 * r + lane];
        if (wave == 0) m.dbuf[192 + lk + 4 * r] = m.Pc[12 * 256 + 64 * r + lane];
      }
    }
    __syncthreads();
    if (wave == 0) {
      for (int i = lane; i < n; i += 64) xk_st_sys(a.corr + i, m.dbuf[i]);
      asm volatile("s_waitcnt vmcnt(0)" ::: "memory");
      if (lane == 0 && a.done_flag) __hip_atomic_store(a.done_flag, a.done_seq, XK_MARKER_ORDER, __HIP_MEMORY_SCOPE_SYSTEM);
    }
  };
  auto store_tile = [&](int I, int J, int lane, const xk_d4 &v, bool both) {
    const int li = lane & 15, lk = lane >> 4, col = 16 * J + li;
    if (col >= n) return;
    double *pb = a.Pout + (size_t)col + (size_t)lk * n;
    double *pm = a.Pout + (size_t)lk + (size_t)col * n;
    const bool whole = 16 * I + 16 <= n;
#pragma unroll
    for (int r = 0; r < 4; ++r) {
      if (whole || 16 * I + lk + 4 * r < n) {
        pb[(size_t)((16 * I + 4 * r) * n)] = v[r];
        if (both) pm[16 * I + 4 * r] = v[r];
      }
    }
  };
  const int nblocks = min(npanels, (na + 15) / 16);
  bool bad = false;
  if (wave == 0) {
    {
      const XkKalLds m(kb);
      const int lane = lane_, li = lane & 15, lk = lane >> 4;
#pragma unroll
      for (int I = 0; I < NB; ++I)
#pragma unroll
        for (int r = 0; r < 4; ++r) m.P0[I * 256 + 64 * r + lane] = ldsym(16 * I + lk + 4 * r, li);
#pragma unroll
      for (int r = 0; r < 4; ++r) {
        m.Pc[64 * r + lane] = ldsym(lk + 4 * r, 192 + li);
        m.Pc[12 * 256 + 64 * r + lane] = ldsym(192 + lk + 4 * r, 192 + li);
      }
    }
    xk_d4 none[NB];
    for (int k = 0; k < nblocks; ++k) {
      const XkKalLds m(xk_opaque(kb));
      int nrows;
      long long *stp = a.dbg ? a.dbg + 2048 + 16 * k : nullptr;
      if (stp && lane_ == 0) stp[0] = wall_clock64();
      if (!fetch(m, k, nrows)) return false;
      if (stp && lane_ == 0) stp[1] = wall_clock64();
      xk_kal_block<false>(m, none, k, nrows, n, a.sigma2, 0, xk_launder(lane_), bad, stp);
    }
    const XkKalLds m(kb);
    const int lane = lane_;
    if (bad && lane == 0) __hip_atomic_store(a.status, 2, __ATOMIC_RELAXED, __HIP_MEMORY_SCOPE_SYSTEM);
    if (a.dbg && lane == 0) a.dbg[2048 + 16 * 31 + 1] = wall_clock64();
    publish(m, lane);
    if (a.dbg && lane == 0) a.dbg[2048 + 16 * 31 + 2] = wall_clock64();
    {
      xk_d4 cc;
#pragma unroll
      for (int r = 0; r < 4; ++r) cc[r] = m.Pc[12 * 256 + 64 * r + lane];
      store_tile(12, 12, lane, cc, false);
    }
    if (a.dbg && lane == 0) a.dbg[2048 + 16 * 31] = wall_clock64();
    return true;
  }
  xk_d4 Pt[NB];
  {
    const XkKalLds m(kb);
    const int lane = lane_, li = lane & 15, lk = lane >> 4;
#pragma unroll
    for (int I = 0; I < NB; ++I) {
#pragma unroll
      for (int r = 0; r < 4; ++r) Pt[I][r] = ldsym(16 * I + lk + 4 * r, 16 * wave + li);
      __builtin_amdgcn_sched_barrier(0);
    }
#pragma unroll
    for (int r = 0; r < 4; ++r) m.Pc[wave * 256 + 64 * r + lane] = ldsym(16 * wave + lk + 4 * r, 192 + li);
  }
  for (int k = 0; k < nblocks; ++k) {
    const XkKalLds m(xk_opaque(kb));
    int nrows;
    if (!fetch(m, k, nrows)) return false;
    long long *stp = (a.dbg && wave == 5) ? a.dbg + 2560 + 16 * k : nullptr;
    xk_kal_block<true>(m, Pt, k, nrows, n, a.sigma2, wave, xk_launder(lane_), bad, stp);
  }
  const XkKalLds m(kb);
  const int lane = lane_;
  publish(m, lane);
#pragma unroll
  for (int I = 0; I < NB; ++I) {
    store_tile(I, wave, lane, Pt[I], false);
    __builtin_amdgcn_sched_barrier(0);
  }
  {
    xk_d4 c, c0t, p0a, p0b;
    const int e = (wave == 1) ? 0 : 0;
    (void)e;
#pragma unroll
    for (int r = 0; r < 4; ++r) {
      c[r] = m.Pc[wave * 256 + 64 * r + lane];
      p0a[r] = m.P0[wave * 256 + 64 * r + lane];
      p0b[r] = m.P0[64 * r + lane];
      c0t[r] = m.Pc[64 * r + lane];
    }
    store_tile(wave, 12, lane, c, true);
    store_tile(wave, 0, lane, p0a, false);
    if (wave == 1) store_tile(0, 0, lane, p0b, false);
    if (wave == 11) store_tile(0, 12, lane, c0t, true);
  }
  return true;
}

template <class G>
__global__ __launch_bounds__(XK_PIPE_THREADS) void xk_caqr_pipe(XkCaqrPipeArgs a) {
  constexpr int RPL = G::RPL, NT = G::NT, NM = G::NM, RM = G::RM, LPC = G::LPC;
  constexpr int LDS_T = 2 * LPC * (RPL + 2), LDS_M = 2 * 16 * (RM + 2), LDS_L = 2 * 16 * (G::RL + 2);
  constexpr int LDS_MAX = LDS_T > LDS_M ? (LDS_T > LDS_L ? LDS_T : LDS_L) : (LDS_M > LDS_L ? LDS_M : LDS_L);
  __shared__ __attribute__((aligned(16))) double ubuf[LDS_MAX];
  __shared__ __attribute__((aligned(16))) double sc[2 * 4];
  __shared__ unsigned s_slot, s_ok;
  __shared__ int rp_pre[XK_PIPE_SLOTS_MAX + 1], rp_rows[LPC * RPL];
  __shared__ __attribute__((aligned(16))) double pfbuf[XK_PIPE_PF ? (XK_PIPE_THREADS / 64) * 24 * 16 : 2];
  constexpr bool KAL = G::COLS <= 192 && G::LPC == 4 && G::RPL <= 40;
  __shared__ __attribute__((aligned(16))) double kbuf[KAL ? XK_KAL_LDS : 2];
  constexpr int HB_OWN = KAL ? 2 : 16 * 1024;
  __shared__ __attribute__((aligned(16))) double hbuf_own[HB_OWN];
  double *hbuf = KAL ? kbuf : hbuf_own;
  constexpr int HB = KAL ? XK_KAL_LDS : HB_OWN;
  unsigned *sync = a.sync, *ab = sync + XP_ABORT * 16;
  const XkPipeArgsPtr ap = (XkPipeArgsPtr)__builtin_amdgcn_kernarg_segment_ptr();
  const unsigned xcc = xk_xcc_id();
  const long long t_entry = a.dbg ? wall_clock64() : 0;
  if (threadIdx.x == 0) {
    const unsigned sl = __hip_atomic_fetch_add(sync + (XP_CENSUS + xcc) * 16, 1u, XK_RLX_AGENT);
    const bool bad = sl >= 32u || gridDim.x != 256u;
    if (bad) { __hip_atomic_store(ab, 3u, XK_RLX_AGENT); a.status[1] = 3; }
    s_slot = sl;
    s_ok = bad ? 0u : 1u;
  }
  __syncthreads();
  if (!s_ok) return;
  const int slot = __builtin_amdgcn_readfirstlane((int)s_slot);
  __syncthreads();
  if (a.test_stall && xcc == 3 && slot == 5) return;
  if (a.dbg && slot >= NT && threadIdx.x == 0) a.dbg[45056 + ((int)xcc * 32 + slot) * 2] = wall_clock64();
#if XK_DATA_POLL
  if (slot >= NT && a.Xnext) {
    const int SSl = 16 * a.C1P, npl = (a.C1 + 15) / 16, nseg = 2 * npl * XK_PIPE_RLS;
    const int nwg = 8 * (32 - NT), wg = (int)xcc * (32 - NT) + (slot - NT), tid = (int)threadIdx.x;
    const double ny = xk_notyet();
    const xk_d2 ny2 = {ny, ny};
    for (int sg = wg; sg < nseg; sg += nwg) {
      const int k = (sg / XK_PIPE_RLS) % npl;
      double *p = a.Xnext + (size_t)sg * SSl;
      for (int e = 256 * k + 2 * tid; e < SSl; e += 2 * XK_PIPE_THREADS) *reinterpret_cast<xk_d2 *>(p + e) = ny2;
    }
    double *pp = a.Xnext + (size_t)nseg * SSl;
    const int n1p = npl * XK_PIPE_RLS * 256;
    for (int e = 2 * (wg * XK_PIPE_THREADS + tid); e < n1p; e += 2 * nwg * XK_PIPE_THREADS) *reinterpret_cast<xk_d2 *>(pp + e) = ny2;
  }
#endif
  if (a.dbg && slot >= NT && threadIdx.x == 0) a.dbg[45056 + ((int)xcc * 32 + slot) * 2 + 1] = wall_clock64();
  bool ok;
  if (slot < NT) {
    int rows_acc;
    const int TR = xk_pipe_rowplan<G>(a, (int)xcc * NT + slot, rp_pre, rp_rows, &rows_acc);
    if (xcc == 0 && slot == 0 && threadIdx.x == 0) __hip_atomic_store(a.status + 2, (a.acc_tag << 15) | min(rows_acc, 0x7fff), __ATOMIC_RELAXED, __HIP_MEMORY_SCOPE_SYSTEM);
    const int nvalid = min(max(rows_acc - ((int)xcc * NT + slot) * TR, 0), TR);
    if (TR == 0) {
      if (threadIdx.x == 0) { __hip_atomic_store(ab, 9u, XK_RLX_AGENT); a.status[1] = 9; }
      ok = false;
    } else if (G::RPLT < G::RPLS && TR <= LPC * G::RPLT) ok = xk_pipe_tile<G, G::RPLT>(ap, (int)xcc, slot, t_entry, ubuf, sc, &s_ok, rp_rows, hbuf, HB, nvalid);
    else if (G::RPLS < RPL && TR <= LPC * G::RPLS) ok = xk_pipe_tile<G, G::RPLS>(ap, (int)xcc, slot, t_entry, ubuf, sc, &s_ok, rp_rows, hbuf, HB, nvalid);
    else ok = xk_pipe_tile<G, RPL>(ap, (int)xcc, slot, t_entry, ubuf, sc, &s_ok, rp_rows, hbuf, HB, nvalid);
  }
  else if (slot < NT + NM) ok = xk_pipe_first<G>(ap, (int)xcc, slot - NT, ubuf, sc, &s_ok, pfbuf);
  else {
    for (int i = (int)xcc * XK_PIPE_THREADS + threadIdx.x; i < XP_WORDS * 16; i += 8 * XK_PIPE_THREADS) a.sync_next[i] = 0u;
    if ((int)xcc < XK_PIPE_NLW) ok = xk_pipe_last<G>(ap, (int)xcc, ubuf, sc, &s_ok);
    else {
      ok = true;
      if constexpr (KAL) {
        if (a.kal) {
          ok = xk_pipe_kalman<G>(ap, (xk_ldsd *)kbuf, &s_ok);
          if (!ok) {
            if (threadIdx.x == 0) __hip_atomic_store(a.status + 1, (int)__hip_atomic_load(ab, XK_RLX_AGENT), __ATOMIC_RELAXED, __HIP_MEMORY_SCOPE_SYSTEM);
            asm volatile("s_waitcnt vmcnt(0)" ::: "memory");
            __syncthreads();
            if (threadIdx.x == 0 && a.done_flag) __hip_atomic_store(a.done_flag, a.done_seq, XK_MARKER_ORDER, __HIP_MEMORY_SCOPE_SYSTEM);
          }
          if (a.dbg && threadIdx.x == 0) a.dbg[2048 + 16 * 31 + 3] = wall_clock64();
          return;
        }
      }
    }
  }
  if (!ok && threadIdx.x == 0) a.status[1] = (int)__hip_atomic_load(ab, XK_RLX_AGENT);
}
```

### x_multi_agent_amd/csrc/xk_compress.hip.h

```cpp
#pragma once
#include <type_traits>

__global__ __launch_bounds__(256) void xk_stack_rows(const double *A, const int *tile_rows, const int *trk_off, int DB, int C1P, int row0, double *T) {
  const int t = blockIdx.x;
  const int nr = 2 * (trk_off[t + 1] - trk_off[t]) - 3, off = row0 + 2 * trk_off[t] - 3 * t, valid = min(tile_rows[t], nr);
  const double *src = A + (size_t)t * DB * C1P;
  double *dst = T + (size_t)off * C1P;
  for (int e = threadIdx.x; e < nr * C1P; e += blockDim.x) dst[e] = (e / C1P < valid) ? src[e] : 0.0;
}

__global__ void xk_mark_done(unsigned long long *p, unsigned long long v) { __hip_atomic_store(p, v, __ATOMIC_RELEASE, __HIP_MEMORY_SCOPE_SYSTEM); }

struct UpdateSpec {
  const double *T;
  long str, stc;
  int c, kdim, col0;
  const double *z;
  long sz;
  const double *rdiag;
  double rscalar;
  const double *S;
  long ssr, ssc;
  const double *Pin;
  double *Pout;
// ... 1 lines not shown
  int cov_update;
  double *corr;
  unsigned long long *done_flag;
  unsigned long long done_seq;
  int tri;
  int naux;
};

struct XkCompressEnv {
  int wt, arity1, chalf, overlap, skip_rejected, persist_dbg, lchalf, adapt, cus, m32;
};
static const XkCompressEnv &compress_env() {
  static const XkCompressEnv e = {env_int("XK_CAQR_WT", 0),       env_int("XK_CAQR_ARITY1", 0),        env_int("XK_CAQR_CHALF", 8),
                                  env_int("XK_CAQR_OVERLAP", 1),  env_int("XK_CAQR_SKIP_REJECTED", 1), env_int("XK_CAQR_PERSIST_DBG", 0),
                                  env_int("XK_CAQR_LCHALF", 0),   env_int("XK_CAQR_ADAPT", 1),         env_int("XK_CAQR_CUS", 256),
                                  env_int("XK_CAQR_M32", 1)};
  return e;
}

static int slot_rows_nominal(const xk_handle *h, int t) {
  if (t < h->K) return 2 * (h->h_trk_off[t + 1] - h->h_trk_off[t]) - 3;
  if (t < h->K + h->K2) return 2 * (h->h_trk2_off[t - h->K + 1] - h->h_trk2_off[t - h->K]) - 3;
  return std::min(h->DB, 2 * h->M - (t - h->K - h->K2) * h->DB);
}
static long split_rows_nominal(const xk_handle *h) {
  long r = 0;
  for (int t = 0; t < h->K + h->K2; ++t) r += slot_rows_nominal(h, t);
  return r;
}

static int pipe_rows_cap(int cols) { return cols <= XkPipeNarrow::COLS ? XkPipeNarrow::ROWS : XkPipeWide::ROWS; }
static bool pipe_queueable(const xk_handle *h, long R, int nslots, int rows_cap) {
  return R >= h->opt_pipe_min_rows && nslots <= XK_PIPE_SLOTS_MAX && R * 4 <= (long)rows_cap * 5 && (h->overflow_rows == 0 || R < h->overflow_rows);
}
static bool kalman_rides(const xk_handle *h) { return h->opt_kalman && h->C1 <= XkPipeNarrow::COLS && h->n <= 206 && h->n_cu == 256; }

static int split_plan(const xk_handle *h) {
  if (!h->d_R2 || !h->opt_slam_split || h->want_full_T) return 0;
  if (h->K + h->K2 > 0) {
    const long R = split_rows_nominal(h) + 2L * h->M;
    if (R <= std::min(h->n, h->CM)) return 3;
  }
  if (h->M <= 0) return 0;
  if (h->K + h->K2 == 0) return 2 * h->M <= h->CM ? 2 : 0;
  if (h->DB != 64 || !h->opt_resident || !h->persist_ok) return 0;
  if (h->n <= 206 || 6 * h->N + 1 > XkPipeWide::COLS) return 0;
  return pipe_queueable(h, split_rows_nominal(h), h->K + h->K2, pipe_rows_cap(6 * h->N + 1)) ? 1 : 0;
}

template <int RPL>
static void launch_merge(xk_handle *h, XkCaqrArgs &a, int groups, int csplit) {
  hipLaunchKernelGGL(HIP_KERNEL_NAME(xk_caqr_merge<RPL>), dim3(groups, csplit), dim3(16 * (16 + a.chalf)), 0, h->stream, a);
}

template <typename F>
static void tile_variant(const xk_handle *h, int rows_max, int tsplit, F f) {
  auto with = [&](auto rpl) { tsplit == 1 ? f(rpl, std::false_type{}) : f(rpl, std::true_type{}); };
  if (h->DB == 64) with(std::integral_constant<int, 16>{});
  else if (rows_max <= 104 && h->opt_tall26) with(std::integral_constant<int, 26>{});
  else with(std::integral_constant<int, 32>{});
}
static void tile_geom(const xk_handle *h, int c0, int &tsplit, int &tchalf, int &tthreads) {
  const int tile_cols = (h->DB == 64) ? 192 : 128;
  const int trail = std::max(0, h->C1 - c0 - 16);
  tsplit = std::max(1, (trail + (tile_cols - 16) - 1) / (tile_cols - 16));
  tchalf = (trail + tsplit - 1) / tsplit;
  tthreads = round_up(4 * (16 + tchalf), 64);
}
static void launch_tile(xk_handle *h, XkCaqrArgs &t) {
  int tsplit, tthreads;
  tile_geom(h, t.c0, tsplit, t.chalf, tthreads);
  const dim3 tgrid(t.ntiles, tsplit), tblock(tthreads);
  tile_variant(h, t.rows_max, tsplit, [&](auto rpl, auto split) {
    hipLaunchKernelGGL(HIP_KERNEL_NAME(xk_caqr_tile<decltype(rpl)::value, decltype(split)::value>), tgrid, tblock, 0, h->stream, t);
  });
}

static int queued(xk_handle *h, const char *what) {
  const hipError_t e = hipGetLastError();
  return e == hipSuccess ? XK_OK : fail(h, XK_EDEVICE, what, e);
}

static int pipe_arm(xk_handle *h, XkCaqrPipeArgs &pa) {
  if (h->xsync_dirty) {
    if (hipMemsetAsync(h->d_xsync, 0, sizeof(unsigned) * 2 * XP_WORDS * 16, h->stream) != hipSuccess) return fail(h, XK_EDEVICE, "sync words");
    if (hipMemsetD32Async((hipDeviceptr_t)h->d_x1, (int)(XK_NOTYET_BITS & 0xffffffffu), 2 * 2 * h->xslab_doubles, h->stream) != hipSuccess) return fail(h, XK_EDEVICE, "slabs");
    h->xsync_dirty = false; h->xsync_phase = 0;
  }
  const size_t np_ = (size_t)(pa.C1 + 15) / 16, strips_ = np_ * XK_PIPE_RLS, x1n = strips_ * 16 * h->C1P;
  double *set = h->d_x1 + (size_t)h->xsync_phase * h->xslab_doubles;
  pa.X1 = set; pa.X2 = set + x1n; pa.X1P = set + 2 * x1n;
  pa.Xnext = h->d_x1 + (size_t)(h->xsync_phase ^ 1) * h->xslab_doubles;
  pa.xnext_doubles = (long)h->xslab_doubles;
  pa.sync = h->d_xsync + (size_t)h->xsync_phase * XP_WORDS * 16;
  pa.sync_next = h->d_xsync + (size_t)(h->xsync_phase ^ 1) * XP_WORDS * 16;
  h->xsync_phase ^= 1;
  if (h->opt_poison) {
    const unsigned seven = 7u;
    if (hipMemcpyAsync(pa.sync + XP_ABORT * 16, &seven, sizeof(unsigned), hipMemcpyHostToDevice, h->stream) != hipSuccess) return fail(h, XK_EDEVICE, "poison");
    if (hipStreamSynchronize(h->stream) != hipSuccess) return fail(h, XK_EDEVICE, "poison");
  }
  pa.dbg = compress_env().persist_dbg ? h->d_pdbg : nullptr;
  pa.test_stall = h->opt_test_stall;
  h->pipe_tag = (h->pipe_tag % 0x7fff) + 1;
  pa.acc_tag = h->pipe_tag;
  return XK_OK;
}

static int launch_pipe_tail(xk_handle *h, bool four, int ccut, int slot0, int nslots, int arity1, int nextra, double *Rout) {
  XkCaqrPipeArgs pa;
  memset(&pa, 0, sizeof(pa));
  pa.A = h->d_A + (size_t)slot0 * h->DB * h->C1P + ccut; pa.tile_rows = h->d_tile_rows + slot0; pa.nslots = nslots; pa.slot_rows = h->DB;
  pa.lead_stride = arity1;
  pa.nextra = nextra; pa.extra_row0 = (long)(h->ntiles_max - slot0) * h->DB;
  pa.Hc = nullptr; pa.hs = 0; pa.nhc = 0;
  pa.C1P = h->C1P; pa.C1 = h->C1 - ccut; pa.Rout = Rout; pa.S = h->d_rs; pa.PB = h->d_rpb;
  pa.status = h->d_status;
  { const int rca = pipe_arm(h, pa); if (rca != XK_OK) return rca; }
  h->pipe_rows_nominal = 0;
  if (four) hipLaunchKernelGGL(xk_caqr_pipe<XkPipeTail4>, dim3(h->n_cu), dim3(XK_PIPE_THREADS), 0, h->stream, pa);
  else hipLaunchKernelGGL(xk_caqr_pipe<XkPipeTail>, dim3(h->n_cu), dim3(XK_PIPE_THREADS), 0, h->stream, pa);
  return queued(h, "caqr tail launch");
}

static int compress_none(xk_handle *h, XkOutcome &o) {
  if (hipMemsetAsync(h->d_R, 0, sizeof(double) * (size_t)h->C1P * h->C1P, h->stream) != hipSuccess) return fail(h, XK_EDEVICE, "R memset");
  o.schedule = XK_SCHED_EMPTY;
  return XK_OK;
}

static int compress_as_built(xk_handle *h, int mode, hipEvent_t mid, XkOutcome &o) {
  const size_t slam_bytes = sizeof(double) * 2 * (size_t)h->M * h->C1P;
  const double *slam_rows = h->d_A + (size_t)(h->K + h->K2) * h->DB * h->C1P;
  if (mode == 3) {
    const int Rt = h->K > 0 ? 2 * h->h_trk_off[h->K] - 3 * h->K : 0;
    if (h->K > 0) hipLaunchKernelGGL(xk_stack_rows, dim3(h->K), dim3(256), 0, h->stream, h->d_A, h->d_tile_rows, h->d_trk_off, h->DB, h->C1P, 0, h->d_R2);
    if (h->K2 > 0)
      hipLaunchKernelGGL(xk_stack_rows, dim3(h->K2), dim3(256), 0, h->stream, h->d_A + (size_t)h->K * h->DB * h->C1P, h->d_tile_rows + h->K, h->d_trk2_off, h->DB,
                         h->C1P, Rt, h->d_R2);
    const long Rall = split_rows_nominal(h);
    if (h->M > 0 && hipMemcpyAsync(h->d_R2 + (size_t)Rall * h->C1P, slam_rows, slam_bytes, hipMemcpyDeviceToDevice, h->stream) != hipSuccess)
      return fail(h, XK_EDEVICE, "SLAM rows");
    h->d_R2_dirty = true;
  } else {
    if (hipMemcpyAsync(h->d_R2 + (size_t)6 * h->N * h->C1P, slam_rows, slam_bytes, hipMemcpyDeviceToDevice, h->stream) != hipSuccess)
      return fail(h, XK_EDEVICE, "SLAM rows");
  }
  if (mid) hipEventRecord(mid, h->stream);
  o.schedule = mode == 3 ? XK_SCHED_SMALL_STACK : XK_SCHED_SLAM_ROWS;
  return queued(h, mode == 3 ? "stack rows" : "SLAM rows");
}

static int compress_single(xk_handle *h, int ntiles, bool sp, hipEvent_t mid, const UpdateSpec *fuse, XkOutcome &o) {
  const int C1s = sp ? 6 * h->N + 1 : h->C1, nslots_p = sp ? h->K + h->K2 : ntiles;
  const bool narrow = C1s <= XkPipeNarrow::COLS;
  const int R_nom = (int)split_rows_nominal(h) + (sp ? 0 : 2 * h->M);
  bool split = false;
  if (narrow && h->opt_split > 0) {
    if (h->split_backoff > 0) --h->split_backoff;
    else if (h->opt_split >= 3) split = true;
    else if (h->opt_split == 2) split = R_nom <= XkPipeNarrow2::ROWS;
    else if (h->acc_ratio > 0.0) split = (long)(h->acc_ratio * 1.02 * R_nom) + 64 <= XkPipeNarrow2::ROWS;
  }
  h->pipe_rows_nominal = R_nom;
  if (!pipe_queueable(h, R_nom, nslots_p, pipe_rows_cap(C1s))) return XK_OK;
  XkCaqrPipeArgs pa;
  memset(&pa, 0, sizeof(pa));
  pa.A = h->d_A; pa.tile_rows = h->d_tile_rows; pa.nslots = nslots_p; pa.slot_rows = 64;
  pa.Hc = h->d_Hc; pa.hs = h->hc_stride; pa.nhc = h->rows_compact ? h->K : 0;
  pa.C1P = h->C1P; pa.C1 = C1s; pa.Rout = sp ? h->d_R2 : h->d_R; pa.S = h->d_rs; pa.PB = h->d_rpb;
  pa.res_col = sp ? h->na : 0;
  pa.status = h->d_status;
  { const int rca = pipe_arm(h, pa); if (rca != XK_OK) return rca; }
  pa.kal = 0; pa.kn = h->n; pa.Pin = nullptr; pa.Pout = nullptr; pa.sigma2 = 0.0; pa.corr = nullptr; pa.ct = nullptr; pa.done_flag = nullptr; pa.done_seq = 0;
  if (fuse && kalman_rides(h) && !fuse->S && !fuse->rdiag && !fuse->naux && fuse->T == h->d_R) {
    pa.kal = 1; pa.Pin = fuse->Pin; pa.Pout = fuse->cov_update ? fuse->Pout : h->d_tmpP; pa.sigma2 = fuse->rscalar; pa.ct = fuse->ct;
    pa.corr = fuse->corr ? fuse->corr : h->d_corr;
    pa.done_flag = fuse->done_flag; pa.done_seq = fuse->done_seq;
  }
  if (sp && h->d_R2_dirty) {
    if (hipMemsetAsync(h->d_R2, 0, sizeof(double) * (size_t)6 * h->N * h->C1P, h->stream) != hipSuccess) return fail(h, XK_EDEVICE, "R2 memset");
    h->d_R2_dirty = false;
  }
  if (split) hipLaunchKernelGGL(xk_caqr_pipe<XkPipeNarrow2>, dim3(h->n_cu), dim3(XK_PIPE_THREADS), 0, h->stream, pa);
  else if (narrow) hipLaunchKernelGGL(xk_caqr_pipe<XkPipeNarrow>, dim3(h->n_cu), dim3(XK_PIPE_THREADS), 0, h->stream, pa);
  else hipLaunchKernelGGL(xk_caqr_pipe<XkPipeWide>, dim3(h->n_cu), dim3(XK_PIPE_THREADS), 0, h->stream, pa);
  if (sp) {
    const int slam0 = h->K + h->K2;
    if (hipMemcpyAsync(h->d_R2 + (size_t)6 * h->N * h->C1P, h->d_A + (size_t)slam0 * h->DB * h->C1P, sizeof(double) * 2 * (size_t)h->M * h->C1P,
                       hipMemcpyDeviceToDevice, h->stream) != hipSuccess)
      return fail(h, XK_EDEVICE, "SLAM rows");
  }
  if (pa.kal && !fuse->cov_update && fuse->Pout != fuse->Pin &&
      hipMemcpyAsync(fuse->Pout, fuse->Pin, sizeof(double) * (size_t)h->n * h->n, hipMemcpyDeviceToDevice, h->stream) != hipSuccess)
    return fail(h, XK_EDEVICE, "prior copy");
  if (mid) hipEventRecord(mid, h->stream);
  const int NTP = 8 * (narrow ? (split ? XkPipeNarrow2::NT : XkPipeNarrow::NT) : XkPipeWide::NT);
  o = {sp ? XK_SCHED_SINGLE_SPLIT : XK_SCHED_SINGLE, pa.kal != 0, split, NTP, 1};
  return queued(h, "caqr launch");
}

struct XkTailPlan { int ccut, half; bool four; };
static XkTailPlan tail_plan(const xk_handle *h, int ntiles, int arity1, int groups1) {
  XkTailPlan p = {0, 0, false};
  std::vector<long> pre((size_t)groups1 + 1, 0);
  for (int g = 0; g < groups1; ++g) {
    long r = 0;
    for (int t = g * arity1; t < std::min(ntiles, (g + 1) * arity1); ++t) {
      const int v = slot_rows_nominal(h, t);
      r += (t % arity1 == 0) ? std::max(v, 32) : v;
    }
    pre[g + 1] = pre[g] + r;
  }
  const long R_nom = pre[groups1];
  if (R_nom < 64 * 8) return p;
  const int cc4 = 16 * std::max(1, (h->C1 - XkPipeTail4::COLS + 15) / 16), cc8 = 16 * ((h->C1 - XkPipeTail::COLS + 15) / 16);
  const int nx = h->C1 - cc4;
  int gh = 0;
  for (int g = 1; g < groups1; ++g)
    if (std::labs(2 * pre[g] - R_nom - nx) < std::labs(2 * pre[gh] - R_nom - nx) || gh == 0) gh = g;
  const long capq = (long)XkPipeTail4::ROWS * 5 / 4;
  if (h->opt_tail != 2 && R_nom * 4 <= (long)XkPipeTail4::ROWS * 5) p = {cc4, 0, true};
  else if (h->opt_tail != 2 && gh > 0 && pre[gh] <= capq && R_nom - pre[gh] + nx <= capq) p = {cc4, gh * arity1, true};
  else if (cc8 >= 16 && R_nom * 4 <= (long)XkPipeTail::ROWS * 5) p = {cc8, 0, false};
  if (p.ccut >= h->C1) p.ccut = 0;
  return p;
}

static int multi_overlapped(xk_handle *h, XkCaqrArgs &a, int arity1, int groups1, const XkTailPlan &tp, hipEvent_t mid, int *launches) {
  const XkCompressEnv &env = compress_env();
  const int ntiles = a.ntiles;
  a.rows_max = std::max(a.rows_max, 32);
  for (int c0 = 0, k = 0; c0 < h->C1; c0 += 16, ++k) {
    const int trail = std::max(0, h->C1 - c0 - 16);
    const int llanes = (h->DB == 64) ? 32 : 16;
    const int lauto = std::min(8, 2 * std::max(1, (trail + 2 * 84 - 1) / (2 * 84)));
    const int lchalf = (h->DB == 64) ? std::min(8, 2 * std::max(1, (env.lchalf ? env.lchalf : lauto) / 2))
                                     : std::min(16, 4 * std::max(1, (env.lchalf ? env.lchalf : 16) / 4));
    const int lsplit = std::max(1, (trail + lchalf - 1) / lchalf);
    const int lead_off = (k & 1) ? 16 : 0;
    if (k == 0) {
      XkCaqrArgs t = a;
      t.c0 = 0; t.stride = 1; t.final_level = 0; t.pin = nullptr; t.pout = h->d_panel[0];
      launch_tile(h, t);
      if (mid) hipEventRecord(mid, h->stream);
    }
    XkCaqrArgs m = a;
    const int per_cu = std::max(1, env.cus / groups1);
    const int mchalf = env.adapt ? std::min(arity1 == 40 ? 16 : 32, std::max(env.chalf, 2 * ((trail + 2 * per_cu - 1) / (2 * per_cu)))) : env.chalf;
    const int msplit = std::max(1, (trail + mchalf - 1) / mchalf);
    m.c0 = c0; m.stride = 1; m.final_level = 0; m.pin = h->d_panel[0]; m.pout = h->d_panel[1]; m.chalf = mchalf;
    m.lead_off = lead_off; m.lead_all = 0; m.pend = (k > 0) ? 1 : 0;
    if (arity1 == 40 && env.m32) hipLaunchKernelGGL(xk_caqr_merge32, dim3(groups1, msplit), dim3(32 * (16 + mchalf)), 0, h->stream, m);
    else if (arity1 == 40) launch_merge<42>(h, m, groups1, msplit);
    else launch_merge<22>(h, m, groups1, msplit);
    ++*launches;
    XkCaqrArgs l = a;
    l.c0 = c0; l.stride = arity1; l.final_level = 1; l.pin = h->d_panel[1]; l.pout = h->d_panel[0]; l.chalf = lchalf;
    l.lead_off = lead_off; l.lead_all = 1; l.pend = 0;
    if (tp.ccut > 0 && c0 + 16 == tp.ccut) {
      launch_merge<20>(h, l, 1, lsplit);
      ++*launches;
      const int ccut = tp.ccut;
      double *const Rtail = h->d_R + (size_t)ccut * h->C1P + ccut;
      int rct;
      if (tp.half > 0) {
        double *Ra = h->d_A + (size_t)h->ntiles_max * h->DB * h->C1P + ccut;
        rct = launch_pipe_tail(h, true, ccut, 0, tp.half, arity1, 0, Ra);
        if (rct == XK_OK) rct = launch_pipe_tail(h, true, ccut, tp.half, ntiles - tp.half, arity1, h->C1 - ccut, Rtail);
        ++*launches;
      } else rct = launch_pipe_tail(h, tp.four, ccut, 0, ntiles, arity1, 0, Rtail);
      if (rct != XK_OK) return rct;
      ++*launches;
      break;
    }
    if (c0 + 16 < h->C1) {
      XkCaqrArgs t = a;
      t.c0 = c0 + 16; t.stride = 1; t.final_level = 0; t.pin = nullptr; t.pout = h->d_panel[0];
      t.hole_stride = arity1; t.lead_off = 16 - lead_off;
// ... 180 lines not shown
```

### x_multi_agent_amd/csrc/xk_handle.hip.h

```cpp
#pragma once

#define XK_STAGE_SLOTS 8
#define XK_PDBG_WORDS 65536

enum XkSchedule {
  XK_SCHED_NONE = 0,
  XK_SCHED_EMPTY,
  XK_SCHED_SLAM_ROWS,
  XK_SCHED_SMALL_STACK,
  XK_SCHED_SINGLE,
  XK_SCHED_SINGLE_SPLIT,
  XK_SCHED_MULTI,
  XK_SCHED_MULTI_TAIL,
};
struct XkOutcome {
  XkSchedule schedule;
  bool fused;
  bool narrow2;
  int leaves, launches;
};
static inline int outcome_R2_mode(const XkOutcome &o) { return o.schedule == XK_SCHED_SINGLE_SPLIT ? 1 : o.schedule == XK_SCHED_SLAM_ROWS ? 2 : o.schedule == XK_SCHED_SMALL_STACK ? 3 : 0; }
static inline void outcome_release_R2(XkOutcome &o) {
  if (o.schedule == XK_SCHED_SINGLE_SPLIT) o.schedule = XK_SCHED_SINGLE;
  else if (o.schedule == XK_SCHED_SLAM_ROWS || o.schedule == XK_SCHED_SMALL_STACK) o.schedule = XK_SCHED_NONE;
}
static inline bool outcome_single(const XkOutcome &o) { return o.schedule == XK_SCHED_SINGLE || o.schedule == XK_SCHED_SINGLE_SPLIT; }
static inline int outcome_status(const XkOutcome &o) {
  return o.schedule == XK_SCHED_NONE || o.schedule == XK_SCHED_MULTI ? 0 : outcome_single(o) ? 2 : o.schedule == XK_SCHED_MULTI_TAIL ? 3 : 4;
}

struct xk_handle {
  int device;
  hipStream_t stream;
  hipStream_t copy_stream;
  hipEvent_t ev_flags, ev_flags_done;
  hipEvent_t ev[16];
  int N, Mmax, Kmax, n, na, C1, C1P, DB, ntiles_max;
  int n_poses, K, M;
  size_t obs_cap;
  double *d_q, *d_p, *d_obs, *d_feat, *d_zlast;
  int *d_trk_off, *d_anchor, *d_tsz;
  double *d_P, *d_Pout;
  double *d_Psnap;
  double *d_Psnap2;
  double *d_fq;
  double *d_chi95, *d_chi90;
  double *d_A;
  double *d_Hc;
  int hc_stride;
  int opt_hlite;
  bool rows_compact;
  int *d_tile_rows;
  double *d_panel[2];
  int *d_inl, *d_inl_s, *d_gn;
  double *d_gam, *d_gam_s, *d_gpf;
  double *d_R;
  double *d_x1;
  size_t xslab_doubles;
  double *d_rs, *d_rpb;
  unsigned *d_xsync;
  int xsync_phase;
  int pipe_rows_nominal;
  int opt_split;
  double acc_ratio;
  int pipe_tag;
  int split_backoff;
  int overflow_rows;
  double *d_R2;
  XkOutcome last;
  int plan;
  bool d_R2_dirty;
  bool want_full_T;
  int opt_slam_split;
  int opt_pipe_min_rows;
  bool tail_capable;
  bool tail_ok;
  int tail_backoff_len;
  int tail_clean, tail_backoff, opt_tail;
  long long *d_pdbg;
  long long *feat_dbg;
  bool attr_slaminit, attr_feat_batch;
  int n_cu;
  bool persist_ok;
  bool fast_capable;
  int fast_giveups, fast_reason;
  int clean_classic, rearm_after;
  int opt_resident, opt_poison, opt_test_stall, opt_tall26;
  int opt_kalman;
  bool compress_deferred;
  int fused_cov_update;
  bool fused_ct_zero;
  std::vector<double> *fused_ct;
  bool fused_pending;
  unsigned long long fused_seq;
  bool xsync_dirty;
  bool have_rows, have_R;
  double sigma_img;
  int CM, LDA;
  double *d_Maug, *d_X, *d_corr, *d_ct, *d_tmpH, *d_tmpS, *d_tmpP, *d_rdiag, *d_tmpz;
  double *h_win;
  bool win_pending;
  bool win_valid;
  unsigned *d_done_cnt;
  unsigned long long done_seq, done_seen, flags_after_seq;
  int *d_status;
  double *h_out;
  double *d_payload;
  double *d_ci;
  double *d_ciws;
  int opt_ci_search;
  double *d_ciw;
  double ci_last_w[8];
  int ci_last_k1, ci_last_iters;
  double *d_ciwr;
  int ci_round_tracks;
  double ci_round_w[8][8];
  int ci_round_k1[8], ci_round_iters[8];
  hipStream_t ci_stream[8];
  hipEvent_t ci_fork, ci_join[8];
  XkFeatBatch *d_batch;
  XkFeatBatch *h_batch;
  int *h_ci_cols;
  double *h_ci_w;
  int *h_trk_off;
  int anchor_max;
  int K2;
  bool ms_built;
  int *d_trk2_off, *h_trk2_off, *d_inl2, *d_gn2;
  double *d_obs2, *d_gpf2, *d_W2, *d_gam2, *d_H1, *d_H2, *d_r1, *d_feat2;
  int *d_csr_i;
  double *d_csr_v;
  size_t csr_cap;
  char *h_stage[XK_STAGE_SLOTS];
  int stage_since_sync;
  size_t stage_bytes;
  int stage_next;
  bool flags_direct;
  bool flags_cached;
  int *h_flag_i;
  double *h_flag_d;
  char *trk_slot;
  int trk_slot_K, trk_slot_nobs;
  bool async_pending;
  XkAuxIn aux_in;
  int aux_staged;
// ... 39 lines not shown
```

### x_multi_agent_amd/engine.py

```python
import ctypes as C
import os

import numpy as np

_HERE = os.path.dirname(os.path.abspath(__file__))
LIB_PATH = os.environ.get("XK_LIB_PATH", os.path.join(_HERE, "libxk.so"))
LAB_LIB_PATH = os.path.join(_HERE, "lab", "libxk.so")
STRICT_LIB_PATH = os.path.join(_HERE, "libxk_strict.so")
_LIBS = {}

c_dp = C.POINTER(C.c_double)
c_ip = C.POINTER(C.c_int)

XK_NSTAGE = 6
STATUS = {0: "XK_OK", 1: "XK_EINVAL", 2: "XK_ESINGULAR", 3: "XK_ENAN", 4: "XK_EDEVICE", 5: "XK_ENOMEM",
          6: "XK_ECAPACITY"}

SYMBOLS = [
    "xk_create", "xk_destroy", "xk_strerror", "xk_last_error", "xk_version", "xk_stream",
    "xk_stage_window", "xk_stage_tracks", "xk_stage_tracks_begin", "xk_stage_tracks_end", "xk_stage_slam", "xk_upload_P", "xk_download_P",
    "xk_msckf_build", "xk_qr_compress", "xk_apply_update", "xk_visual_update_staged", "xk_visual_update",
    "xk_apply_update_dense", "xk_apply_ci", "xk_fuse_ci_msckf", "xk_fuse_ci_slam", "xk_multi_slam_match", "xk_msckf_ci_track",
    "xk_ci_round_device", "xk_ci_round_weights", "xk_ci_solve_weights", "xk_ci_last_weights", "xk_cov_congruence", "xk_cov_propagate",
    "xk_stage_msckf_slam", "xk_msckf_slam_results", "xk_init_msckf_slam_features", "xk_init_standard_slam_features",
    "xk_payload_doubles", "xk_pack_payload", "xk_bench_staged", "xk_run_steps",
    "xk_apply_ci_resident", "xk_snapshot_P", "xk_caqr_status", "xk_set_option", "xk_build_compress_async", "xk_build_compress_update_async", "xk_build_compress_update_pass_async", "xk_fetch_flags",
    "xk_stage_range", "xk_stage_sun_angle", "xk_fetch_aux_flags", "xk_aux_rows",
    "xk_pr_create", "xk_pr_destroy", "xk_pr_vlad_bytes", "xk_pr_size", "xk_pr_compute_vlad", "xk_pr_add_keyframe",
    "xk_pr_find_candidate", "xk_pr_keyframe", "xk_pr_copy_keyframe", "xk_pr_knn_match",
    "xk_pr_essential_ransac", "xk_pr_essential_hypotheses",
    "xk_trk_create", "xk_trk_destroy", "xk_trk_undistort", "xk_trk_fundamental_ransac", "xk_trk_fundamental_hypotheses",
    "xk_trk_filter_matches",
    "xk_trk_klt_setup", "xk_trk_klt_levels", "xk_trk_push_image", "xk_trk_track", "xk_trk_klt_level",
]


LAB_SYMBOLS = ["xk_is_lab", "xk_probe_fp64_peak", "xk_debug_persist_stamps", "xk_debug_feature_points"]


class XkTiming(C.Structure):
    _fields_ = [("total_ms", C.c_float), ("stage_ms", C.c_float * XK_NSTAGE),
                ("stage_launches", C.c_int * XK_NSTAGE), ("stage_name", (C.c_char * 32) * XK_NSTAGE),
                ("n", C.c_int), ("c1", C.c_int), ("k_tracks", C.c_int), ("rows_stacked", C.c_int),
                ("n_leaf", C.c_int), ("n_levels", C.c_int)]


class XkError(RuntimeError):
    def __init__(self, status, what, detail=""):
        super().__init__(f"{what}: {STATUS.get(status, status)} {detail}".strip())
        self.status = status


def _load(path):
    if not os.path.exists(path):
        raise ImportError(f"{path} not found: build it with `python -m x_multi_agent_amd.build` "
                          "(hipcc --offload-arch=gfx950); there is no CPU fallback")
    try:
        import torch
    except ImportError:
        pass
    L = C.CDLL(path)
    L.xk_strerror.restype = C.c_char_p
    L.xk_last_error.restype = C.c_char_p
    L.xk_last_error.argtypes = [C.c_void_p]
    L.xk_stream.restype = C.c_void_p
    L.xk_stream.argtypes = [C.c_void_p]
    L.xk_payload_doubles.restype = C.c_long
    return L


def lib(lab=False, path=None):
    p = os.path.abspath(path if path else (LAB_LIB_PATH if lab else LIB_PATH))
    if p not in _LIBS:
        _LIBS[p] = _load(p)
    return _LIBS[p]


def _d(a):
    a = np.ascontiguousarray(a, dtype=np.float64)
    return a, a.ctypes.data_as(c_dp)


def _i(a):
    a = np.ascontiguousarray(a, dtype=np.int32)
    return a, a.ctypes.data_as(c_ip)


def _f(a):
    a = np.asfortranarray(a, dtype=np.float64)
    return a, a.ctypes.data_as(c_dp)


class Engine:

    def __init__(self, n_poses_max, n_feat_max, k_max, device=0, lab=False, lib_path=None):
        self.L = lib(lab, lib_path)
        self.h = C.c_void_p()
        rc = self.L.xk_create(C.c_int(device), C.c_int(n_poses_max), C.c_int(n_feat_max), C.c_int(k_max),
                              C.byref(self.h))
        if rc != 0:
            raise XkError(rc, "xk_create")
        self.N, self.M, self.K = n_poses_max, n_feat_max, k_max
        self.n = 15 + 6 * n_poses_max + 3 * n_feat_max

    def close(self):
        if self.h:
            self.L.xk_destroy(self.h)
            self.h = C.c_void_p()

# ... 252 lines not shown
        k = len(tracks)
        self.K2 = k
        if k == 0:
            self._chk(self.L.xk_stage_msckf_slam(self.h, None, None, C.c_int(0)), "xk_stage_msckf_slam")
            return
        off, offp = _i(np.concatenate([[0], np.cumsum([len(t) for t in tracks])]))
        obs, obsp = _d(np.concatenate([np.asarray(t, float).reshape(-1, 2) for t in tracks]))
        self._chk(self.L.xk_stage_msckf_slam(self.h, offp, obsp, C.c_int(k)), "xk_stage_msckf_slam")

    def msckf_slam_results(self):
        k = getattr(self, "K2", 0)
        m = max(3 * k, 1)
        inl = np.zeros(max(k, 1), np.int32)
        gam = np.zeros(max(k, 1))
        H1 = np.zeros((m, self.n), order="F")
        H2 = np.zeros((m, m), order="F")
        r1, f = np.zeros(m), np.zeros(m)
        self._chk(self.L.xk_msckf_slam_results(self.h, inl.ctypes.data_as(c_ip), gam.ctypes.data_as(c_dp),
                                               H1.ctypes.data_as(c_dp), C.c_int(m), H2.ctypes.data_as(c_dp), C.c_int(m),
                                               r1.ctypes.data_as(c_dp), f.ctypes.data_as(c_dp)), "xk_msckf_slam_results")
        return dict(inlier=inl[:k], gamma=gam[:k], H1=np.ascontiguousarray(H1[:3 * k]), H2=np.ascontiguousarray(H2[:3 * k, :3 * k]),
                    r1=r1[:3 * k], features=f[:3 * k])

    def init_msckf_slam_features(self, n_features, correction, sigma_img):
        k = getattr(self, "K2", 0)
        corr, corrp = _d(correction)
        out = np.zeros(max(3 * k, 1))
        self._chk(self.L.xk_init_msckf_slam_features(self.h, C.c_int(n_features), corrp, C.c_double(sigma_img),
                                                     out.ctypes.data_as(c_dp)), "xk_init_msckf_slam_features")
        return out[:3 * k]

    def init_standard_slam_features(self, n_features, k, sigma_img, sigma_rho_0):
        self._chk(self.L.xk_init_standard_slam_features(self.h, C.c_int(n_features), C.c_int(k), C.c_double(sigma_img),
                                                        C.c_double(sigma_rho_0)), "xk_init_standard_slam_features")

    def cov_congruence(self, J):
        if isinstance(J, tuple):
            rp, ci, v = J
        else:
            J = np.asarray(J, dtype=np.float64)
            nz = [np.nonzero(row)[0] for row in J]
            rp = np.concatenate([[0], np.cumsum([len(z) for z in nz])])
            ci = np.concatenate(nz) if len(nz) else np.zeros(0, int)
            v = np.concatenate([J[i, z] for i, z in enumerate(nz)]) if len(nz) else np.zeros(0)
        rp_, rpp = _i(rp)
        ci_, cip = _i(ci if len(ci) else [0])
        v_, vp = _d(v if len(v) else [0.0])
        self._chk(self.L.xk_cov_congruence(self.h, rpp, cip, vp, C.c_int(int(rp_[-1]))), "xk_cov_congruence")

    def cov_propagate(self, f_d, q_d):
        f, fp = _f(f_d)
        q, qp = _f(q_d)
        self._chk(self.L.xk_cov_propagate(self.h, fp, C.c_int(15), qp, C.c_int(15)), "xk_cov_propagate")

    def ci_round_device(self, payloads_ptr, payload_stride, world, self_rank, tracks_ptr, n_tracks, track_len,
                        n_poses_valid, self_track, sigma_img, ci_msckf_w, want_corrections=False):
        tl, tlp = _i(np.asarray(track_len, dtype=np.int32).ravel())
        nv, nvp = _i(np.asarray(n_poses_valid, dtype=np.int32).ravel())
        st, stp = _i(np.asarray(self_track, dtype=np.int32).ravel())
        nf = C.c_int()
        corr = np.zeros((max(n_tracks, 1), self.n)) if want_corrections else None
        self._chk(self.L.xk_ci_round_device(
            self.h, C.cast(C.c_void_p(payloads_ptr), c_dp), C.c_long(payload_stride), C.c_int(world), C.c_int(self_rank),
            C.cast(C.c_void_p(tracks_ptr), c_dp), C.c_int(n_tracks), tlp, nvp, stp, C.c_double(sigma_img),
            C.c_double(ci_msckf_w), C.byref(nf), corr.ctypes.data_as(c_dp) if want_corrections else None),
            "xk_ci_round_device")
        return nf.value, (corr[:nf.value] if want_corrections else None)

    def bench_staged(self, sigma_img, warmup, steps):
        t = XkTiming()
        self._chk(self.L.xk_bench_staged(self.h, C.c_double(sigma_img), C.c_int(warmup), C.c_int(steps),
                                         C.byref(t)), "xk_bench_staged")
        return dict(total_ms=t.total_ms,
                    stages={t.stage_name[s].value.decode(): dict(ms=t.stage_ms[s], launches=t.stage_launches[s])
                            for s in range(XK_NSTAGE)},
                    n=t.n, c1=t.c1, k_tracks=t.k_tracks, rows_stacked=t.rows_stacked, n_leaf=t.n_leaf,
                    n_levels=t.n_levels)

    def caqr_status(self):
        v = [C.c_int() for _ in range(4)]
        self._chk(self.L.xk_caqr_status(self.h, *[C.byref(x) for x in v]), "xk_caqr_status")
        return dict(schedule=v[0].value, armed=bool(v[1].value), giveups=v[2].value, last_reason=v[3].value)

    def set_option(self, name, value):
        self._chk(self.L.xk_set_option(self.h, name.encode(), C.c_int(int(value))), "xk_set_option")

    def probe_fp64_peak(self, use_mfma=True):
        t = C.c_double()
        self._chk(self.L.xk_probe_fp64_peak(self.h, C.c_int(int(use_mfma)), C.byref(t)), "xk_probe_fp64_peak")
        return t.value

    def debug_feature_points(self):
        K = max(self._K, 1)
        gpf, it = np.zeros((K, 3)), np.zeros(K, dtype=np.int32)
        self._chk(self.L.xk_debug_feature_points(self.h, gpf.ctypes.data_as(c_dp), it.ctypes.data_as(c_ip), C.c_int(self._K)),
                  "xk_debug_feature_points")
        return gpf[:self._K], it[:self._K]

    def payload_doubles(self):
        return int(self.L.xk_payload_doubles(C.c_int(self.N), C.c_int(self.M)))

    def pack_payload_into(self, agent_id, timestamp, dyn16, device_ptr=None):
        d, dp = _d(dyn16)
        ptr = c_dp()
        dst = C.cast(C.c_void_p(device_ptr), c_dp) if device_ptr else None
        self._chk(self.L.xk_pack_payload(self.h, C.c_double(agent_id), C.c_double(timestamp), dp, dst,
                                         C.byref(ptr)), "xk_pack_payload")
        return C.cast(ptr, C.c_void_p).value

    def stage_range(self, range_m, img_pt, facet, sigma_range):
        f, fp = _i(facet)
        self._chk(self.L.xk_stage_range(self.h, C.c_double(range_m), C.c_double(img_pt[0]), C.c_double(img_pt[1]), fp,
                                        C.c_double(sigma_range)), "xk_stage_range")

    def stage_sun_angle(self, q_xyzw, x_angle, y_angle, calib=None):
        q, qp = _d(q_xyzw)
        cp = None
        if calib is not None:
            cb, cp = _d(calib)
        self._chk(self.L.xk_stage_sun_angle(self.h, qp, C.c_double(x_angle), C.c_double(y_angle), cp), "xk_stage_sun_angle")

    def fetch_aux_flags(self):
        inl, gam = C.c_int(), C.c_double()
        self._chk(self.L.xk_fetch_aux_flags(self.h, C.byref(inl), C.byref(gam)), "xk_fetch_aux_flags")
        return inl.value, gam.value

    def aux_rows(self):
        H = np.zeros((3, self.n), order="F")
        res, rd, rows = np.zeros(3), np.zeros(3), C.c_int()
        self._chk(self.L.xk_aux_rows(self.h, H.ctypes.data_as(c_dp), C.c_int(3), res.ctypes.data_as(c_dp), rd.ctypes.data_as(c_dp),
                                     C.byref(rows)), "xk_aux_rows")
        m = rows.value
        return np.ascontiguousarray(H[:m]), res[:m].copy(), rd[:m].copy()

    def run_steps(self, sigma_img, steps):
        self._chk(self.L.xk_run_steps(self.h, C.c_double(sigma_img), C.c_int(steps)), "xk_run_steps")


def LabEngine(*a, **kw):
    return Engine(*a, lab=True, **kw)
```

Before: 2910 updates/s.

## Add 15-column CAQR panel width option and exclude residual column from panel count

Templates the pipelined CAQR tile, first, last and Kalman stages on a panel width and adds runtime fields for panel width and residual-column count. The single-launch path now excludes the residual column when counting panels, which can drop a final partial panel, and can use 15-wide panels when the pivot column count is a multiple of 15. This trims wasted lanes and sync epochs in the last panel, at the cost of extra per-row guards and doubled kernel instantiations. The default panel width stays 16 unless an option or environment variable selects 15 or auto.

```diff
diff --git a/include/xk.h b/include/xk.h
--- a/include/xk.h
+++ b/include/xk.h
@@ -207,6 +207,8 @@
 
 int xk_caqr_status(const xk_handle *h, int *schedule, int *armed, int *giveups, int *last_reason);
 
+int xk_caqr_panel_width(const xk_handle *h);
+
 int xk_set_option(xk_handle *h, const char *name, int value);
 
 #ifdef __cplusplus
diff --git a/x_multi_agent_amd/csrc/xk_api.hip b/x_multi_agent_amd/csrc/xk_api.hip
--- a/x_multi_agent_amd/csrc/xk_api.hip
+++ b/x_multi_agent_amd/csrc/xk_api.hip
@@ -160,6 +160,7 @@
     h->opt_test_stall = env_int("XK_CAQR_TEST_STALL", 0);
     h->opt_tall26 = env_int("XK_CAQR_TALL26", 1);
     h->opt_kalman = env_int("XK_PIPE_KALMAN", 1);
+    h->opt_panel_width = env_int("XK_PIPE_PW", XK_PIPE_PW_DEFAULT);
     if (h->opt_split >= 0) h->opt_split = env_int("XK_PIPE_SPLIT", 1);
     if (!h->fast_capable && h->DB == 64 && h->C1 <= XkPipeWide::COLS) {
       snprintf(h->err, sizeof(h->err), "single-launch CAQR unavailable on device %d: %s; the multi-launch schedule serves every update",
@@ -2268,6 +2269,11 @@
   else if (!strcmp(name, "caqr_rearm")) h->rearm_after = value;
   else if (!strcmp(name, "caqr_tail")) h->opt_tail = value;
   else if (!strcmp(name, "slam_split")) h->opt_slam_split = value;
+  else if (!strcmp(name, "caqr_panel_width")) {
+    if (value != 0 && value != 15 && value != 16) return fail(h, XK_EINVAL, "xk_set_option: caqr_panel_width is 0, 15 or 16");
+    if (value == 15 && h->na % 15 != 0) return fail(h, XK_EINVAL, "xk_set_option: caqr_panel_width 15 needs pivot columns that are a multiple of 15");
+    h->opt_panel_width = value;
+  }
   else if (!strcmp(name, "ci_weight_search")) {
     if (value != 0 && value != 1) return fail(h, XK_EINVAL, "xk_set_option: ci_weight_search is 0 or 1");
     h->opt_ci_search = value;
@@ -2292,6 +2298,8 @@
   if (last_reason) *last_reason = h->fast_reason;
   return XK_OK;
 }
+
+extern "C" int xk_caqr_panel_width(const xk_handle *h) { return h ? h->pipe_pw : 0; }
 
 #ifdef XK_LAB
 extern "C" int xk_is_lab(void) { return 1; }
diff --git a/x_multi_agent_amd/csrc/xk_caqr_pipe.hip.h b/x_multi_agent_amd/csrc/xk_caqr_pipe.hip.h
--- a/x_multi_agent_amd/csrc/xk_caqr_pipe.hip.h
+++ b/x_multi_agent_amd/csrc/xk_caqr_pipe.hip.h
@@ -121,6 +121,8 @@
   int nextra;
   long extra_row0;
   int C1P, C1;
+  int pw;
+  int nres;
   double *Rout;
   double *S;
   double *PB;
@@ -148,6 +150,9 @@
   __builtin_memcpy(&a, (const void *)ap, sizeof(a));
   return a;
 }
+__host__ __device__ __forceinline__ int xk_pipe_npanels(int C1, int nres, int pw) { return (C1 - nres + pw - 1) / pw; }
+__host__ __device__ __forceinline__ int xk_pipe_nsteps(int C1, int nres, int pw, int c0) { return (C1 - nres - c0 < pw) ? C1 - nres - c0 : pw; }
+__host__ __device__ __forceinline__ int xk_pipe_slab_panels(int C1) { return (C1 + 15) / 16; }
 
 __device__ __forceinline__ void xk_pipe_arrive(unsigned *cnt) {
   (void)__hip_atomic_fetch_add(cnt, 1u, XK_ARRIVE_ORDER, __HIP_MEMORY_SCOPE_AGENT);
@@ -458,7 +463,7 @@
   return max(TR, 1);
 }
 
-template <class G, int RPL>
+template <class G, int RPL, int PW>
 __device__ __noinline__ bool xk_pipe_tile(XkPipeArgsPtr ap, int xcc, int slot, long long t_entry, double *ubuf, double *sc, unsigned *s_ok,
                                           const int *myrows, double *hbuf, int hcap_doubles, int nvalid) {
   constexpr int NT = G::NT, LPC = G::LPC, NPH = G::NPH, GS = 16 / NPH, ARRD = XK_PIPE_ARRD;
@@ -469,7 +474,8 @@
   const int j = xcc * NT + slot;
   const int cabs = tid / LPC, part_ = tid % LPC;
   const bool mine = cabs < a.C1;
-  const int npanels = (a.C1 + 15) / 16;
+  constexpr int pw = PW;
+  const int npanels = xk_pipe_npanels(a.C1, a.nres, pw);
   const bool stamp = a.dbg && xcc == 0 && slot == 1 && tid == 0;
   double b[RPL];
   if (a.nhc > 0) {
@@ -593,13 +599,13 @@
   double *myPB = a.PB + (size_t)j * 256;
   if (stamp) { a.dbg[1536] = t_entry; a.dbg[1537] = wall_clock64(); }
   for (int k = 0; k < npanels; ++k) {
-    const int c0 = 16 * k;
+    const int c0 = pw * k;
     const int part = xk_launder(part_);
     const int rel = xk_launder(cabs) - c0;
-    const int nsteps = (a.C1 - c0 < 16) ? a.C1 - c0 : 16;
-    const bool full = nsteps == 16;
+    const int nsteps = xk_pipe_nsteps(a.C1, a.nres, pw, c0);
+    const bool full = nsteps == pw;
     const int wrel = (tid >> 6) * (64 / LPC) - c0;
-    const bool hot = wrel <= 0 && wrel > -(64 / LPC);
+    const bool hot = wrel < nsteps && wrel > -(64 / LPC);
     const bool pub = mine && part == 0 && rel >= 0;
     const unsigned epoch = (unsigned)(k + 1);
     if (stamp) { a.dbg[16 * k + 0] = wall_clock64(); a.dbg[16 * k + 8] = clock64(); }
@@ -612,14 +618,15 @@
       auto hook = [&]() { xk_pipe_arrive(sync + (XP_TQ_CNT + (q - 1) * 8 + xcc) * 16); if (a.dbg && k == 0 && q == 1) a.dbg[47104 + j] = wall_clock64(); };
       xk_pipe_range<LPC, xk_pbn<NPH>(q), xk_pbn<NPH>(q + 1), (q > 0 ? xk_pbn<NPH>(q) + ARRD : -1), RPL>(b, nullptr, rel, mine, false, part, nsteps, ubuf, sc, full, hook);
       if (pub) {
-        if (rel < 16) {
+        if (rel < pw) {
           double *pb = xk_opaque(myPB + xk_blk(rel, 0));
 #pragma unroll
-          for (int r = xk_pbn<NPH>(q); r < xk_pbn<NPH>(q + 1); ++r) pb[r * 4] = (r > rel) ? 0.0 : b[r];
+          for (int r = xk_pbn<NPH>(q); r < xk_pbn<NPH>(q + 1); ++r) pb[r * 4] = (r > rel || r >= nsteps) ? 0.0 : b[r];
         } else {
           double *ps = xk_opaque(myS + xk_blk(cabs, 0));
 #pragma unroll
-          for (int r = xk_pbn<NPH>(q); r < xk_pbn<NPH>(q + 1); ++r) ps[r * 4] = b[r];
+          for (int r = xk_pbn<NPH>(q); r < xk_pbn<NPH>(q + 1); ++r)
+            if (r < pw) ps[r * 4] = b[r];
         }
       }
       if (stamp && q < 4) a.dbg[16 * k + 1 + q] = wall_clock64();
@@ -644,10 +651,11 @@
     if (!xk_pipe_wait(sync + (XP_MB_CNT + xcc) * 16, (unsigned)G::NM * epoch, ab, 2u, s_ok)) return false;
     if (stamp) a.dbg[16 * k + 6] = wall_clock64();
     XK_INV_LOC();
-    if (mine && rel >= 16 && part == 0) {
+    if (mine && rel >= pw && part == 0) {
       const double *ps = xk_opaque(myS + xk_blk(cabs, 0));
 #pragma unroll
-      for (int r = 0; r < 16; ++r) b[r] = XK_LD_LOC(ps + r * 4);
+      for (int r = 0; r < 16; ++r)
+        if (r < pw) b[r] = XK_LD_LOC(ps + r * 4);
     }
     if (stamp) {
       double sink = 0;
@@ -664,7 +672,7 @@
   asm volatile("s_mov_b32 m0, %1\n\tglobal_load_lds_dwordx4 %0, off sc1" ::"v"(src), "s"(lds_byte) : "memory", "m0");
 }
 
-template <class G>
+template <class G, int PW>
 __device__ __noinline__ bool xk_pipe_first(XkPipeArgsPtr ap, int xcc, int item, double *ubuf, double *sc, unsigned *s_ok, double *pfbuf) {
   constexpr int NT = G::NT, NM = G::NMG, RM = G::RM, NP = 16, NPH = G::NPH, GS = 16 / NPH, NCL = G::NCL, NCM = G::NCM;
   constexpr int NG = G::NG, NTG = G::NTG;
@@ -673,7 +681,9 @@
   const int tid = threadIdx.x;
   const int cidx_ = tid / NP, part_ = tid & (NP - 1);
   const bool panel = cidx_ < 16;
-  const int npanels = (a.C1 + 15) / 16;
+  constexpr int pw = PW;
+  const int npanels = xk_pipe_npanels(a.C1, a.nres, pw);
+  const bool rowok = part_ < pw;
   const int grp = NG > 1 ? item / NM : 0;
   item -= grp * NM;
   const int nts = NG > 1 ? min(NTG, NT - grp * NTG) : NT;
@@ -682,16 +692,16 @@
   const size_t SS = (size_t)16 * a.C1P;
   const bool stamp = a.dbg && xcc == 0 && item == 0 && tid == 0;
   for (int k = 0; k < npanels; ++k) {
-    const int c0 = 16 * k, trail = max(0, a.C1 - c0 - 16);
+    const int c0 = pw * k, trail = max(0, a.C1 - c0 - pw);
     const int cidx = xk_launder(cidx_), part = xk_launder(part_);
     const int mh = min(32, 4 * ((trail + 4 * NM * NCM - 1) / (4 * NM * NCM))), mch = mh * NCM;
     const bool active = item == 0 || item * mch < trail;
-    const int col = panel ? c0 + cidx : c0 + 16 + item * mch + (cidx - 16);
+    const int col = panel ? c0 + cidx : c0 + pw + item * mch + (cidx - 16);
     const int col2 = col + mh;
-    const bool mine = active && col < a.C1 && (panel || cidx - 16 < mh);
+    const bool mine = active && col < a.C1 && (panel ? cidx < pw : cidx - 16 < mh);
     const bool mine2 = NCM > 1 && active && !panel && cidx - 16 < mh && col2 < a.C1;
-    const int nsteps = (a.C1 - c0 < 16) ? a.C1 - c0 : 16;
-    const bool full = nsteps == 16;
+    const int nsteps = xk_pipe_nsteps(a.C1, a.nres, pw, c0);
+    const bool full = nsteps == pw;
     const unsigned epoch = (unsigned)(k + 1);
     const size_t slab = (size_t)k * XK_PIPE_RLS + xcc * NG + grp;
     double b[RM], b2[NCM > 1 ? RM : 2];
@@ -704,18 +714,18 @@
     if (k >= 1 && has_pending) {
 #if XK_DATA_POLL
       double pb1[1] = {0.0}, pb2[1] = {0.0};
-      if (!xk_poll_slots<1>(pb1, a.X2 + pslab * SS + xk_blk(min(col, a.C1P - 1), part), 0, mine, ab, 4u)) *s_ok = 0u;
+      if (!xk_poll_slots<1>(pb1, a.X2 + pslab * SS + xk_blk(min(col, a.C1P - 1), part), 0, mine && rowok, ab, 4u)) *s_ok = 0u;
       if constexpr (NCM > 1) {
-        if (!xk_poll_slots<1>(pb2, a.X2 + pslab * SS + xk_blk(min(col2, a.C1P - 1), part), 0, mine2, ab, 4u)) *s_ok = 0u;
+        if (!xk_poll_slots<1>(pb2, a.X2 + pslab * SS + xk_blk(min(col2, a.C1P - 1), part), 0, mine2 && rowok, ab, 4u)) *s_ok = 0u;
       }
       __syncthreads();
       if (*s_ok == 0u) return false;
-      if (mine) b[0] = pb1[0];
-      if constexpr (NCM > 1) b2[0] = mine2 ? pb2[0] : 0.0;
+      if (mine && rowok) b[0] = pb1[0];
+      if constexpr (NCM > 1) b2[0] = (mine2 && rowok) ? pb2[0] : 0.0;
       if (a.dbg && tid == 0) a.dbg[4096 + ((xcc * NG + grp) * NM + item) * 32 + k] = wall_clock64();
 #else
       if (!xk_pipe_wait(sync + (XP_P_CNT + k - 1) * 16, (unsigned)lsplit_prev, ab, 4u, s_ok)) return false;
-      if (mine) b[0] = xk_ld_sc1(a.X2 + pslab * SS + xk_blk(col, part));
+      if (mine && rowok) b[0] = xk_ld_sc1(a.X2 + pslab * SS + xk_blk(col, part));
 #endif
     }
 #pragma unroll
@@ -724,7 +734,7 @@
 #pragma unroll
       for (int s = 1; s < RM; ++s) b2[s] = 0.0;
 #if !XK_DATA_POLL
-      if (k >= 1 && has_pending && mine2) b2[0] = xk_ld_sc1(a.X2 + pslab * SS + xk_blk(col2, part));
+      if (k >= 1 && has_pending && mine2 && rowok) b2[0] = xk_ld_sc1(a.X2 + pslab * SS + xk_blk(col2, part));
 #endif
     }
     double *g02 = a.S + (size_t)base * SS + xk_blk(min(col2, a.C1P - 1), part);
@@ -738,7 +748,7 @@
     int loaded = 0;
     constexpr bool PF = XK_PIPE_PF && NG == 1 && NCM == 1 && NPH == 4 && NT <= 24 && xk_pbn<NPH>(1) == 4 && xk_pbn<NPH>(2) == 8 && xk_pbn<NPH>(3) == 12;
     const int ln = tid & 63, cid4 = cidx & ~3;
-    const int wcol = panel ? c0 + cid4 : c0 + 16 + item * mch + (cid4 - 16);
+    const int wcol = panel ? c0 + cid4 : c0 + pw + item * mch + (cid4 - 16);
     const bool wv_ok = active && (panel || cid4 - 16 < mh) && wcol < a.C1;
     double *pfw = pfbuf + (size_t)(tid >> 6) * (24 * 16);
     const unsigned pfw_lds = (unsigned)__builtin_amdgcn_readfirstlane((int)(unsigned)(size_t)pfw);
@@ -781,7 +791,7 @@
             }
           }
         } else {
-          if (active && mine && part >= xk_pbn<NPH>(loaded) && part < xk_pbn<NPH>(av)) {
+          if (active && mine && rowok && part >= xk_pbn<NPH>(loaded) && part < xk_pbn<NPH>(av)) {
             double *g = xk_opaque(g0);
 #pragma unroll
             for (int s = 1; s <= NTG; ++s)
@@ -789,7 +799,7 @@
           }
         }
         if constexpr (NCM > 1) {
-          if (mine2 && part >= xk_pbn<NPH>(loaded) && part < xk_pbn<NPH>(av)) {
+          if (mine2 && rowok && part >= xk_pbn<NPH>(loaded) && part < xk_pbn<NPH>(av)) {
             double *g = xk_opaque(g02);
 #pragma unroll
             for (int s = 1; s <= NTG; ++s)
@@ -826,7 +836,7 @@
       phase(std::integral_constant<int, 6>{}); phase(std::integral_constant<int, 7>{});
     }
     if (!ok) return false;
-    if (mine) {
+    if (mine && rowok) {
       if (!panel) {
         double *g = xk_opaque(g0);
 #pragma unroll
@@ -836,7 +846,7 @@
       if (x1_mine && part >= xk_pbn<NPH>(NPH - 1)) xk_st_sc1(x1, (panel && part > cidx) ? 0.0 : b[0]);
     }
     if constexpr (NCM > 1) {
-      if (mine2) {
+      if (mine2 && rowok) {
         double *g = xk_opaque(g02);
 #pragma unroll
         for (int s = 1; s <= NTG; ++s)
@@ -856,7 +866,7 @@
   return true;
 }
 
-template <class G>
+template <class G, int PW>
 __device__ __noinline__ bool xk_pipe_last(XkPipeArgsPtr ap, int lidx, double *ubuf, double *sc, unsigned *s_ok) {
   constexpr int NP = 16, RL = G::RL, NPH = G::NPH, GS = 16 / NPH, NCL = G::NCL, NM = G::NM;
   const XkCaqrPipeArgs a = xk_pipe_args(ap);
@@ -864,20 +874,22 @@
   const int tid = threadIdx.x;
   const int cidx_ = tid / NP, part_ = tid & (NP - 1);
   const bool panel = cidx_ < 16;
-  const int npanels = (a.C1 + 15) / 16;
+  constexpr int pw = PW;
+  const int npanels = xk_pipe_npanels(a.C1, a.nres, pw);
+  const bool rowok = part_ < pw;
   const bool stamp = a.dbg && lidx == 0 && tid == 0;
   const size_t SS = (size_t)16 * a.C1P;
   for (int k = 0; k < npanels; ++k) {
-    const int c0 = 16 * k, trail = max(0, a.C1 - c0 - 16);
+    const int c0 = pw * k, trail = max(0, a.C1 - c0 - pw);
     int ncl, lchalf, lsplit;
     xk_pipe_lastcut(trail, NCL, ncl, lchalf, lsplit);
     if (lidx >= lsplit || lidx >= XK_PIPE_NLW) continue;
     const int cidx = xk_launder(cidx_), part = xk_launder(part_);
-    const int col = panel ? c0 + cidx : c0 + 16 + lidx * lchalf + (cidx - 16);
+    const int col = panel ? c0 + cidx : c0 + pw + lidx * lchalf + (cidx - 16);
     const int col2 = col + XK_PIPE_NLW * lchalf;
-    const bool mine = col < a.C1 && (panel || cidx - 16 < lchalf);
+    const bool mine = col < a.C1 && (panel ? cidx < pw : cidx - 16 < lchalf);
     const bool mine2 = ncl > 1 && !panel && cidx - 16 < lchalf && col2 < a.C1;
-    const int nsteps = (a.C1 - c0 < 16) ? a.C1 - c0 : 16;
+    const int nsteps = xk_pipe_nsteps(a.C1, a.nres, pw, c0);
     const double *src = panel ? a.X1P + (size_t)k * XK_PIPE_RLS * 256 + xk_blk(cidx, part) : a.X1 + (size_t)k * XK_PIPE_RLS * SS + xk_blk(col, part);
     const double *src2 = a.X1 + (size_t)k * XK_PIPE_RLS * SS + xk_blk(min(col2, a.C1P - 1), part);
     const size_t sstep = panel ? 256 : SS;
@@ -891,7 +903,7 @@
       if (!ok || nsteps <= xk_pbn<NPH>(q)) return;
 #if XK_DATA_POLL
       {
-        const bool rows_q = part >= xk_pbn<NPH>(q) && part < xk_pbn<NPH>(q + 1);
+        const bool rows_q = rowok && part >= xk_pbn<NPH>(q) && part < xk_pbn<NPH>(q + 1);
         bool got = xk_poll_slots<RL>(b, src, sstep, rows_q && mine, ab, 5u);
         if (got && ncl > 1) got = xk_poll_slots<RL>(b2, src2, SS, rows_q && mine2, ab, 5u);
         if (!got) *s_ok = 0u;
@@ -907,7 +919,7 @@
         const int av = xk_pipe_wait_phases(sync + (XP_X1_CNT + k) * 16, XK_CAQR_MAXP * 16, q, NPH, 8u * NM, ab, 5u, s_ok);
         if (av == 0) { ok = false; return; }
         if (stamp && q < 4) a.dbg[1024 + 16 * k + 2 * q] = wall_clock64();
-        if (part >= xk_pbn<NPH>(loaded) && part < xk_pbn<NPH>(av)) {
+        if (rowok && part >= xk_pbn<NPH>(loaded) && part < xk_pbn<NPH>(av)) {
           if (mine) {
 #pragma unroll
             for (int s = 0; s < RL; ++s) b[s] = xk_ld_sc1(src + s * sstep);
@@ -933,24 +945,25 @@
     auto rout = [&](size_t at, double v) { if (a.kal) xk_st_sc1(a.Rout + at, v); else a.Rout[at] = v; };
     if (mine) {
       if (panel) {
-        if (lidx == 0 && c0 + part < a.C1) rout((size_t)(c0 + part) * a.C1P + xk_pipe_srccol(a, col), (part > cidx) ? 0.0 : b[0]);
+        if (lidx == 0 && part < nsteps) rout((size_t)(c0 + part) * a.C1P + xk_pipe_srccol(a, col), (part > cidx) ? 0.0 : b[0]);
       } else {
-        if (k + 1 < npanels) {
+        if (k + 1 < npanels && rowok) {
           double *dst = a.X2 + (size_t)k * XK_PIPE_RLS * SS + xk_blk(col, part);
 #pragma unroll
           for (int s = 1; s < RL; ++s) xk_st_sc1(dst + s * SS, b[s]);
         }
-        if (c0 + part < a.C1) rout((size_t)(c0 + part) * a.C1P + xk_pipe_srccol(a, col), b[0]);
+        if (part < nsteps) rout((size_t)(c0 + part) * a.C1P + xk_pipe_srccol(a, col), b[0]);
       }
     }
     if (mine2) {
-      if (k + 1 < npanels) {
+      if (k + 1 < npanels && rowok) {
         double *dst = a.X2 + (size_t)k * XK_PIPE_RLS * SS + xk_blk(col2, part);
 #pragma unroll
         for (int s = 1; s < RL; ++s) xk_st_sc1(dst + s * SS, b2[s]);
       }
-      if (c0 + part < a.C1) rout((size_t)(c0 + part) * a.C1P + xk_pipe_srccol(a, col2), b2[0]);
-    }
+      if (part < nsteps) rout((size_t)(c0 + part) * a.C1P + xk_pipe_srccol(a, col2), b2[0]);
+    }
+    if (a.nres && k + 1 == npanels && lidx == 0 && tid == 0) rout((size_t)(a.C1 - 1) * a.C1P + xk_pipe_srccol(a, a.C1 - 1), 0.0);
     asm volatile("s_waitcnt vmcnt(0)" ::: "memory");
     __syncthreads();
     if (tid == 0) {
@@ -1032,7 +1045,7 @@
   for (int r = 0; r < 4; ++r) { m.Pc[wave * 256 + 64 * r + lane] = c12[r]; if (!REG) m.Pc[12 * 256 + 64 * r + lane] = ccc[r]; }
 }
 template <bool REG>
-__device__ __forceinline__ void xk_kal_block(const XkKalLds &m, xk_d4 (&Pt)[XK_KAL_NB], int k, int nrows, int n, double sigma2, int wave, int lane,
+__device__ __forceinline__ void xk_kal_block(const XkKalLds &m, xk_d4 (&Pt)[XK_KAL_NB], int kt, int nrows, int n, double sigma2, int wave, int lane,
                                              bool &bad, long long *stp) {
 #define XK_KSTAMP(i) do { if (stp && lane == 0) stp[i] = wall_clock64(); } while (0)
   constexpr int NB = XK_KAL_NB, TLD = XK_KAL_TLD;
@@ -1050,7 +1063,7 @@
       else w0 = __builtin_amdgcn_mfma_f64_16x16x4f64(ac[q], bc[q], w0, 0, 0, 0);                                          \
     }                                                                                                                     \
   }
-  switch (k) {
+  switch (kt) {
     case 0: XK_KAL_WTILE(0) [[fallthrough]];
     case 1: XK_KAL_WTILE(1) [[fallthrough]];
     case 2: XK_KAL_WTILE(2) [[fallthrough]];
@@ -1074,7 +1087,7 @@
   xk_d4 W = w0 + w1;
   {
     xk_d4 x = {0, 0, 0, 0};
-    if (wave >= k) {
+    if (wave >= kt) {
 #pragma unroll
       for (int q = 0; q < 4; ++q) x = __builtin_amdgcn_mfma_f64_16x16x4f64(ta[16 * wave + 4 * q], m.Pc[wave * 256 + 64 * q + lane], x, 0, 0, 0);
     }
@@ -1106,7 +1119,7 @@
   XK_KSTAMP(4);
   if (REG && wave == 11) {
     xk_d4 W12 = {0, 0, 0, 0};
-    for (int w = k; w < 13; ++w)
+    for (int w = kt; w < 13; ++w)
 #pragma unroll
       for (int r = 0; r < 4; ++r) W12[r] += m.part[w * 256 + 64 * r + lane];
     if (li == XK_KAL_DC - 192) {
@@ -1121,7 +1134,7 @@
   XK_KSTAMP(5);
   if (!REG) {
     xk_d4 S = {0, 0, 0, 0};
-    for (int J = k; J < 13; ++J)
+    for (int J = kt; J < 13; ++J)
 #pragma unroll
       for (int r = 0; r < 4; ++r) S[r] += m.Sp[J * 288 + 64 * r + lane];
 #pragma unroll
@@ -1156,22 +1169,24 @@
 #undef XK_KSTAMP
 }
 
-template <class G>
+template <class G, int PW>
 __device__ __noinline__ bool xk_pipe_kalman(XkPipeArgsPtr ap, xk_ldsd *kb, unsigned *s_ok) {
   constexpr int NB = XK_KAL_NB, TLD = XK_KAL_TLD, NCL = G::NCL;
   const XkCaqrPipeArgs a = xk_pipe_args(ap);
   unsigned *sync = a.sync, *ab = sync + XP_ABORT * 16;
   const int tid = threadIdx.x, lane_ = tid & 63, wave = __builtin_amdgcn_readfirstlane(tid >> 6);
-  const int n = a.kn, na = a.C1 - 1, npanels = (a.C1 + 15) / 16;
+  constexpr int pw = PW;
+  const int n = a.kn, na = a.C1 - 1, npanels = xk_pipe_npanels(a.C1, a.nres, pw);
   auto ldsym = [&](int row, int col) {
     if (col == XK_KAL_DC) return (a.ct && row < n) ? -a.ct[row] : 0.0;
     return (row < n && col < n) ? 0.5 * (a.Pin[(size_t)row + (size_t)col * n] + a.Pin[(size_t)col + (size_t)row * n]) : 0.0;
   };
-  auto fetch = [&](const XkKalLds &m, int k, int &nrows) -> bool {
-    const int c0 = 16 * k;
-    nrows = min(16, na - c0);
+  auto fetch = [&](const XkKalLds &m, int k, int &nrows, int &kt) -> bool {
+    const int c0 = pw * k;
+    nrows = min(pw, na - c0);
+    kt = (15 + c0) >> 4;
     int ncl, lchalf, lsplit;
-    xk_pipe_lastcut(max(0, a.C1 - c0 - 16), NCL, ncl, lchalf, lsplit);
+    xk_pipe_lastcut(max(0, a.C1 - c0 - pw), NCL, ncl, lchalf, lsplit);
     if (!xk_pipe_wait(sync + (XP_R_CNT + k) * 16, (unsigned)min(XK_PIPE_NLW, lsplit), ab, 8u, s_ok)) return false;
     double tv[5];
 #pragma unroll
@@ -1218,7 +1233,7 @@
       }
     }
   };
-  const int nblocks = min(npanels, (na + 15) / 16);
+  const int nblocks = npanels;
   bool bad = false;
   if (wave == 0) {
     {
@@ -1237,12 +1252,12 @@
     xk_d4 none[NB];
     for (int k = 0; k < nblocks; ++k) {
       const XkKalLds m(xk_opaque(kb));
-      int nrows;
+      int nrows, kt;
       long long *stp = a.dbg ? a.dbg + 2048 + 16 * k : nullptr;
       if (stp && lane_ == 0) stp[0] = wall_clock64();
-      if (!fetch(m, k, nrows)) return false;
+      if (!fetch(m, k, nrows, kt)) return false;
       if (stp && lane_ == 0) stp[1] = wall_clock64();
-      xk_kal_block<false>(m, none, k, nrows, n, a.sigma2, 0, xk_launder(lane_), bad, stp);
+      xk_kal_block<false>(m, none, kt, nrows, n, a.sigma2, 0, xk_launder(lane_), bad, stp);
     }
     const XkKalLds m(kb);
     const int lane = lane_;
@@ -1274,10 +1289,10 @@
   }
   for (int k = 0; k < nblocks; ++k) {
     const XkKalLds m(xk_opaque(kb));
-    int nrows;
-    if (!fetch(m, k, nrows)) return false;
+    int nrows, kt;
+    if (!fetch(m, k, nrows, kt)) return false;
     long long *stp = (a.dbg && wave == 5) ? a.dbg + 2560 + 16 * k : nullptr;
-    xk_kal_block<true>(m, Pt, k, nrows, n, a.sigma2, wave, xk_launder(lane_), bad, stp);
+    xk_kal_block<true>(m, Pt, kt, nrows, n, a.sigma2, wave, xk_launder(lane_), bad, stp);
   }
   const XkKalLds m(kb);
   const int lane = lane_;
@@ -1306,8 +1321,9 @@
   return true;
 }
 
-template <class G>
+template <class G, int PW = 16>
 __global__ __launch_bounds__(XK_PIPE_THREADS) void xk_caqr_pipe(XkCaqrPipeArgs a) {
+  static_assert(PW == 15 || PW == 16, "panels of 15 or 16 columns");
   constexpr int RPL = G::RPL, NT = G::NT, NM = G::NM, RM = G::RM, LPC = G::LPC;
   constexpr int LDS_T = 2 * LPC * (RPL + 2), LDS_M = 2 * 16 * (RM + 2), LDS_L = 2 * 16 * (G::RL + 2);
   constexpr int LDS_MAX = LDS_T > LDS_M ? (LDS_T > LDS_L ? LDS_T : LDS_L) : (LDS_M > LDS_L ? LDS_M : LDS_L);
@@ -1341,14 +1357,14 @@
   if (a.dbg && slot >= NT && threadIdx.x == 0) a.dbg[45056 + ((int)xcc * 32 + slot) * 2] = wall_clock64();
 #if XK_DATA_POLL
   if (slot >= NT && a.Xnext) {
-    const int SSl = 16 * a.C1P, npl = (a.C1 + 15) / 16, nseg = 2 * npl * XK_PIPE_RLS;
+    const int SSl = 16 * a.C1P, npl = xk_pipe_slab_panels(a.C1), nseg = 2 * npl * XK_PIPE_RLS;
     const int nwg = 8 * (32 - NT), wg = (int)xcc * (32 - NT) + (slot - NT), tid = (int)threadIdx.x;
     const double ny = xk_notyet();
     const xk_d2 ny2 = {ny, ny};
     for (int sg = wg; sg < nseg; sg += nwg) {
       const int k = (sg / XK_PIPE_RLS) % npl;
       double *p = a.Xnext + (size_t)sg * SSl;
-      for (int e = 256 * k + 2 * tid; e < SSl; e += 2 * XK_PIPE_THREADS) *reinterpret_cast<xk_d2 *>(p + e) = ny2;
+      for (int e = 64 * ((PW * k) >> 2) + 2 * tid; e < SSl; e += 2 * XK_PIPE_THREADS) *reinterpret_cast<xk_d2 *>(p + e) = ny2;
     }
     double *pp = a.Xnext + (size_t)nseg * SSl;
     const int n1p = npl * XK_PIPE_RLS * 256;
@@ -1365,19 +1381,19 @@
     if (TR == 0) {
       if (threadIdx.x == 0) { __hip_atomic_store(ab, 9u, XK_RLX_AGENT); a.status[1] = 9; }
       ok = false;
-    } else if (G::RPLT < G::RPLS && TR <= LPC * G::RPLT) ok = xk_pipe_tile<G, G::RPLT>(ap, (int)xcc, slot, t_entry, ubuf, sc, &s_ok, rp_rows, hbuf, HB, nvalid);
-    else if (G::RPLS < RPL && TR <= LPC * G::RPLS) ok = xk_pipe_tile<G, G::RPLS>(ap, (int)xcc, slot, t_entry, ubuf, sc, &s_ok, rp_rows, hbuf, HB, nvalid);
-    else ok = xk_pipe_tile<G, RPL>(ap, (int)xcc, slot, t_entry, ubuf, sc, &s_ok, rp_rows, hbuf, HB, nvalid);
-  }
-  else if (slot < NT + NM) ok = xk_pipe_first<G>(ap, (int)xcc, slot - NT, ubuf, sc, &s_ok, pfbuf);
+    } else if (G::RPLT < G::RPLS && TR <= LPC * G::RPLT) ok = xk_pipe_tile<G, G::RPLT, PW>(ap, (int)xcc, slot, t_entry, ubuf, sc, &s_ok, rp_rows, hbuf, HB, nvalid);
+    else if (G::RPLS < RPL && TR <= LPC * G::RPLS) ok = xk_pipe_tile<G, G::RPLS, PW>(ap, (int)xcc, slot, t_entry, ubuf, sc, &s_ok, rp_rows, hbuf, HB, nvalid);
+    else ok = xk_pipe_tile<G, RPL, PW>(ap, (int)xcc, slot, t_entry, ubuf, sc, &s_ok, rp_rows, hbuf, HB, nvalid);
+  }
+  else if (slot < NT + NM) ok = xk_pipe_first<G, PW>(ap, (int)xcc, slot - NT, ubuf, sc, &s_ok, pfbuf);
   else {
     for (int i = (int)xcc * XK_PIPE_THREADS + threadIdx.x; i < XP_WORDS * 16; i += 8 * XK_PIPE_THREADS) a.sync_next[i] = 0u;
-    if ((int)xcc < XK_PIPE_NLW) ok = xk_pipe_last<G>(ap, (int)xcc, ubuf, sc, &s_ok);
+    if ((int)xcc < XK_PIPE_NLW) ok = xk_pipe_last<G, PW>(ap, (int)xcc, ubuf, sc, &s_ok);
     else {
       ok = true;
       if constexpr (KAL) {
         if (a.kal) {
-          ok = xk_pipe_kalman<G>(ap, (xk_ldsd *)kbuf, &s_ok);
+          ok = xk_pipe_kalman<G, PW>(ap, (xk_ldsd *)kbuf, &s_ok);
           if (!ok) {
             if (threadIdx.x == 0) __hip_atomic_store(a.status + 1, (int)__hip_atomic_load(ab, XK_RLX_AGENT), __ATOMIC_RELAXED, __HIP_MEMORY_SCOPE_SYSTEM);
             asm volatile("s_waitcnt vmcnt(0)" ::: "memory");
diff --git a/x_multi_agent_amd/csrc/xk_compress.hip.h b/x_multi_agent_amd/csrc/xk_compress.hip.h
--- a/x_multi_agent_amd/csrc/xk_compress.hip.h
+++ b/x_multi_agent_amd/csrc/xk_compress.hip.h
@@ -107,12 +107,14 @@
 }
 
 static int pipe_arm(xk_handle *h, XkCaqrPipeArgs &pa) {
+  if (h->pipe_pw_armed != 0 && h->pipe_pw_armed != pa.pw) h->xsync_dirty = true;
+  h->pipe_pw_armed = pa.pw;
   if (h->xsync_dirty) {
     if (hipMemsetAsync(h->d_xsync, 0, sizeof(unsigned) * 2 * XP_WORDS * 16, h->stream) != hipSuccess) return fail(h, XK_EDEVICE, "sync words");
     if (hipMemsetD32Async((hipDeviceptr_t)h->d_x1, (int)(XK_NOTYET_BITS & 0xffffffffu), 2 * 2 * h->xslab_doubles, h->stream) != hipSuccess) return fail(h, XK_EDEVICE, "slabs");
     h->xsync_dirty = false; h->xsync_phase = 0;
   }
-  const size_t np_ = (size_t)(pa.C1 + 15) / 16, strips_ = np_ * XK_PIPE_RLS, x1n = strips_ * 16 * h->C1P;
+  const size_t np_ = (size_t)xk_pipe_slab_panels(pa.C1), strips_ = np_ * XK_PIPE_RLS, x1n = strips_ * 16 * h->C1P;
   double *set = h->d_x1 + (size_t)h->xsync_phase * h->xslab_doubles;
   pa.X1 = set; pa.X2 = set + x1n; pa.X1P = set + 2 * x1n;
   pa.Xnext = h->d_x1 + (size_t)(h->xsync_phase ^ 1) * h->xslab_doubles;
@@ -140,9 +142,11 @@
   pa.nextra = nextra; pa.extra_row0 = (long)(h->ntiles_max - slot0) * h->DB;
   pa.Hc = nullptr; pa.hs = 0; pa.nhc = 0;
   pa.C1P = h->C1P; pa.C1 = h->C1 - ccut; pa.Rout = Rout; pa.S = h->d_rs; pa.PB = h->d_rpb;
+  pa.pw = 16; pa.nres = 0;
   pa.status = h->d_status;
   { const int rca = pipe_arm(h, pa); if (rca != XK_OK) return rca; }
   h->pipe_rows_nominal = 0;
+  h->pipe_pw = 16;
   if (four) hipLaunchKernelGGL(xk_caqr_pipe<XkPipeTail4>, dim3(h->n_cu), dim3(XK_PIPE_THREADS), 0, h->stream, pa);
   else hipLaunchKernelGGL(xk_caqr_pipe<XkPipeTail>, dim3(h->n_cu), dim3(XK_PIPE_THREADS), 0, h->stream, pa);
   return queued(h, "caqr tail launch");
@@ -176,6 +180,17 @@
   return queued(h, mode == 3 ? "stack rows" : "SLAM rows");
 }
 
+static int pipe_panel_width(const xk_handle *h, int na) {
+#if XK_PIPE_PF
+  return 16;
+#else
+  const bool legal15 = na > 0 && na % 15 == 0;
+  if (h->opt_panel_width == 16 || !legal15) return 16;
+  if (h->opt_panel_width == 15) return 15;
+  return (na + 14) / 15 <= (na + 15) / 16 ? 15 : 16;
+#endif
+}
+
 static int compress_single(xk_handle *h, int ntiles, bool sp, hipEvent_t mid, const UpdateSpec *fuse, XkOutcome &o) {
   const int C1s = sp ? 6 * h->N + 1 : h->C1, nslots_p = sp ? h->K + h->K2 : ntiles;
   const bool narrow = C1s <= XkPipeNarrow::COLS;
@@ -195,6 +210,7 @@
   pa.Hc = h->d_Hc; pa.hs = h->hc_stride; pa.nhc = h->rows_compact ? h->K : 0;
   pa.C1P = h->C1P; pa.C1 = C1s; pa.Rout = sp ? h->d_R2 : h->d_R; pa.S = h->d_rs; pa.PB = h->d_rpb;
   pa.res_col = sp ? h->na : 0;
+  pa.nres = 1; pa.pw = pipe_panel_width(h, C1s - 1);
   pa.status = h->d_status;
   { const int rca = pipe_arm(h, pa); if (rca != XK_OK) return rca; }
   pa.kal = 0; pa.kn = h->n; pa.Pin = nullptr; pa.Pout = nullptr; pa.sigma2 = 0.0; pa.corr = nullptr; pa.ct = nullptr; pa.done_flag = nullptr; pa.done_seq = 0;
@@ -207,9 +223,14 @@
     if (hipMemsetAsync(h->d_R2, 0, sizeof(double) * (size_t)6 * h->N * h->C1P, h->stream) != hipSuccess) return fail(h, XK_EDEVICE, "R2 memset");
     h->d_R2_dirty = false;
   }
-  if (split) hipLaunchKernelGGL(xk_caqr_pipe<XkPipeNarrow2>, dim3(h->n_cu), dim3(XK_PIPE_THREADS), 0, h->stream, pa);
-  else if (narrow) hipLaunchKernelGGL(xk_caqr_pipe<XkPipeNarrow>, dim3(h->n_cu), dim3(XK_PIPE_THREADS), 0, h->stream, pa);
-  else hipLaunchKernelGGL(xk_caqr_pipe<XkPipeWide>, dim3(h->n_cu), dim3(XK_PIPE_THREADS), 0, h->stream, pa);
+  auto launch = [&](auto geom) {
+    using G = decltype(geom);
+    if (pa.pw == 15) hipLaunchKernelGGL(HIP_KERNEL_NAME(xk_caqr_pipe<G, 15>), dim3(h->n_cu), dim3(XK_PIPE_THREADS), 0, h->stream, pa);
+    else hipLaunchKernelGGL(HIP_KERNEL_NAME(xk_caqr_pipe<G, 16>), dim3(h->n_cu), dim3(XK_PIPE_THREADS), 0, h->stream, pa);
+  };
+  if (split) launch(XkPipeNarrow2{});
+  else if (narrow) launch(XkPipeNarrow{});
+  else launch(XkPipeWide{});
   if (sp) {
     const int slam0 = h->K + h->K2;
     if (hipMemcpyAsync(h->d_R2 + (size_t)6 * h->N * h->C1P, h->d_A + (size_t)slam0 * h->DB * h->C1P, sizeof(double) * 2 * (size_t)h->M * h->C1P,
@@ -220,6 +241,7 @@
       hipMemcpyAsync(fuse->Pout, fuse->Pin, sizeof(double) * (size_t)h->n * h->n, hipMemcpyDeviceToDevice, h->stream) != hipSuccess)
     return fail(h, XK_EDEVICE, "prior copy");
   if (mid) hipEventRecord(mid, h->stream);
+  h->pipe_pw = pa.pw;
   const int NTP = 8 * (narrow ? (split ? XkPipeNarrow2::NT : XkPipeNarrow::NT) : XkPipeWide::NT);
   o = {sp ? XK_SCHED_SINGLE_SPLIT : XK_SCHED_SINGLE, pa.kal != 0, split, NTP, 1};
   return queued(h, "caqr launch");
diff --git a/x_multi_agent_amd/csrc/xk_handle.hip.h b/x_multi_agent_amd/csrc/xk_handle.hip.h
--- a/x_multi_agent_amd/csrc/xk_handle.hip.h
+++ b/x_multi_agent_amd/csrc/xk_handle.hip.h
@@ -2,6 +2,9 @@
 
 #define XK_STAGE_SLOTS 8
 #define XK_PDBG_WORDS 65536
+#ifndef XK_PIPE_PW_DEFAULT
+#define XK_PIPE_PW_DEFAULT 16
+#endif
 
 enum XkSchedule {
   XK_SCHED_NONE = 0,
@@ -61,6 +64,9 @@
   unsigned *d_xsync;
   int xsync_phase;
   int pipe_rows_nominal;
+  int opt_panel_width;
+  int pipe_pw;
+  int pipe_pw_armed;
   int opt_split;
   double acc_ratio;
   int pipe_tag;
diff --git a/x_multi_agent_amd/engine.py b/x_multi_agent_amd/engine.py
--- a/x_multi_agent_amd/engine.py
+++ b/x_multi_agent_amd/engine.py
@@ -24,7 +24,7 @@
     "xk_ci_round_device", "xk_ci_round_weights", "xk_ci_solve_weights", "xk_ci_last_weights", "xk_cov_congruence", "xk_cov_propagate",
     "xk_stage_msckf_slam", "xk_msckf_slam_results", "xk_init_msckf_slam_features", "xk_init_standard_slam_features",
     "xk_payload_doubles", "xk_pack_payload", "xk_bench_staged", "xk_run_steps",
-    "xk_apply_ci_resident", "xk_snapshot_P", "xk_caqr_status", "xk_set_option", "xk_build_compress_async", "xk_build_compress_update_async", "xk_build_compress_update_pass_async", "xk_fetch_flags",
+    "xk_apply_ci_resident", "xk_snapshot_P", "xk_caqr_status", "xk_caqr_panel_width", "xk_set_option", "xk_build_compress_async", "xk_build_compress_update_async", "xk_build_compress_update_pass_async", "xk_fetch_flags",
     "xk_stage_range", "xk_stage_sun_angle", "xk_fetch_aux_flags", "xk_aux_rows",
     "xk_pr_create", "xk_pr_destroy", "xk_pr_vlad_bytes", "xk_pr_size", "xk_pr_compute_vlad", "xk_pr_add_keyframe",
     "xk_pr_find_candidate", "xk_pr_keyframe", "xk_pr_copy_keyframe", "xk_pr_knn_match",
@@ -443,6 +443,9 @@
         self._chk(self.L.xk_caqr_status(self.h, *[C.byref(x) for x in v]), "xk_caqr_status")
         return dict(schedule=v[0].value, armed=bool(v[1].value), giveups=v[2].value, last_reason=v[3].value)
 
+    def caqr_panel_width(self):
+        return int(self.L.xk_caqr_panel_width(self.h))
+
     def set_option(self, name, value):
         self._chk(self.L.xk_set_option(self.h, name.encode(), C.c_int(int(value))), "xk_set_option")
 
```

Measured after the change: 2895 updates/s. Within noise of the previous version (-0.5%).
